# aledima00/sldm-gnn

Measured on NVIDIA B200. Metric: sageblock_fwd_bwd_edges_per_sec, higher is better.
Workload: dtype f32

## Files before the change

### include/sldm_sage.h

```cpp
#ifndef SLDM_SAGE_H_
#define SLDM_SAGE_H_

#include <stddef.h>
#include <stdint.h>

#ifdef __cplusplus
extern "C" {
#endif

#define SLDM_ABI_VERSION 1

#define SLDM_OK            0
#define SLDM_EINVAL        1
#define SLDM_ESHAPE        2
#define SLDM_ECUDA         3
#define SLDM_EWORKSPACE    4
#define SLDM_EUNSUPPORTED  5
#define SLDM_ENODEVICE     6

typedef void* sldm_stream_t;

int         sldm_abi_version(void);
const char* sldm_last_error(void);
int64_t     sldm_launch_count(void);
int         sldm_device_sm_count(int* out_sms);

#define SLDM_HUB_DEGREE 256
#define SLDM_HUB_CHUNK  2048

enum {
  SLDM_CSR_META = 0, SLDM_CSR_ROWPTR_DST = 1, SLDM_CSR_COL_SRC = 2,
  SLDM_CSR_ROWPTR_SRC = 3, SLDM_CSR_COL_DST = 4, SLDM_CSR_HUB_DST = 5,
  SLDM_CSR_HUB_SRC = 6, SLDM_CSR_TOTAL = 7
};
int     sldm_csr_layout(int64_t N, int64_t E, int64_t* out8);
int64_t sldm_csr_workspace_bytes(int64_t N, int64_t E);
int     sldm_csr_build(const int64_t* edge_index, int64_t E, int64_t N,
                       int32_t* csr, void* workspace, int64_t workspace_bytes,
                       sldm_stream_t stream);

int     sldm_csr_status_async(const int32_t* csr, int32_t* status_host_pinned, sldm_stream_t stream);

int     sldm_csr_build_pairs(const int64_t* edge_src, const int64_t* edge_dst, int64_t E, int64_t N,
                             int32_t* csr, void* workspace, int64_t workspace_bytes,
                             sldm_stream_t stream);

int64_t sldm_segment_workspace_bytes(int64_t N, int64_t E, int32_t F);
int     sldm_segment_reduce(const float* src, int64_t N, int32_t F,
                            const int32_t* csr, int64_t E, int32_t transpose,
                            int32_t mean, const float* addend, float* out,
                            void* workspace, int64_t workspace_bytes,
                            sldm_stream_t stream);

int64_t sldm_sage_project_workspace_bytes(int64_t N, int32_t Fin, int32_t Fout);
int     sldm_sage_project_forward(const float* agg, const float* x, int64_t N,
                                  int32_t Fin, int32_t Fout,
                                  const float* W_l, const float* b_l, const float* W_r,
                                  const float* ln_w, const float* ln_b,
                                  float eps, float slope,
                                  float* out, float* xhat_out, float* rstd_out,
                                  void* workspace, int64_t workspace_bytes,
                                  sldm_stream_t stream);

int64_t sldm_sage_layer_fwd_workspace_bytes(int64_t N, int64_t E, int32_t Fin, int32_t Fout);
int     sldm_sage_layer_forward(const float* x, int64_t N, int32_t Fin, int32_t Fout,
                                const int32_t* csr, int64_t E,
                                const float* W_l, const float* b_l, const float* W_r,
                                const float* ln_w, const float* ln_b,
                                float eps, float slope,
                                float* out, float* agg, float* xhat_out, float* rstd_out,
                                void* workspace, int64_t workspace_bytes,
                                sldm_stream_t stream);

int64_t sldm_sage_layer_bwd_workspace_bytes(int64_t N, int64_t E, int32_t Fin, int32_t Fout);
int     sldm_sage_layer_backward(const float* dout, const float* x, const float* agg,
                                 const float* xhat, const float* rstd,
                                 int64_t N, int32_t Fin, int32_t Fout,
                                 const int32_t* csr, int64_t E,
                                 const float* W_l, const float* W_r,
                                 const float* ln_w, const float* ln_b, float slope,
                                 float* dx, float* dW_l, float* db_l, float* dW_r,
                                 float* dln_w, float* dln_b,
                                 float* dz, float* dagg, float* dxroot,
                                 void* workspace, int64_t workspace_bytes,
                                 sldm_stream_t stream);

#define SLDM_BWD_STAGE_LN     1
#define SLDM_BWD_STAGE_DGRAD  2
#define SLDM_BWD_STAGE_WGRAD  4
#define SLDM_BWD_STAGE_GATHER 8
#define SLDM_BWD_STAGE_ALL    15
int     sldm_sage_layer_backward_stages(const float* dout, const float* x, const float* agg,
                                        const float* xhat, const float* rstd,
                                        int64_t N, int32_t Fin, int32_t Fout,
                                        const int32_t* csr, int64_t E,
                                        const float* W_l, const float* W_r,
                                        const float* ln_w, const float* ln_b, float slope,
                                        float* dx, float* dW_l, float* db_l, float* dW_r,
                                        float* dln_w, float* dln_b,
                                        float* dz, float* dagg, float* dxroot,
                                        void* workspace, int64_t workspace_bytes,
                                        sldm_stream_t stream, int32_t stages);

int sldm_sage_bf16_supported(int32_t Fin, int32_t Fout);
int sldm_segment_mean_bf16(const void* src, int64_t N, int32_t F, const int32_t* csr, int64_t E, void* out,
                           void* workspace, int64_t workspace_bytes, sldm_stream_t stream);
int sldm_sage_project_forward_bf16(const void* agg, const void* x, int64_t N, int32_t Fin, int32_t Fout,
                                   const float* W_l, const float* b_l, const float* W_r,
                                   const float* ln_w, const float* ln_b, float eps, float slope,
                                   void* out, float* xhat_out, float* rstd_out,
                                   void* workspace, int64_t workspace_bytes, sldm_stream_t stream);
int sldm_sage_layer_forward_bf16(const void* x, int64_t N, int32_t Fin, int32_t Fout,
                                 const int32_t* csr, int64_t E,
                                 const float* W_l, const float* b_l, const float* W_r,
                                 const float* ln_w, const float* ln_b, float eps, float slope,
                                 void* out, void* agg, float* xhat_out, float* rstd_out,
                                 void* workspace, int64_t workspace_bytes, sldm_stream_t stream);
int sldm_sage_layer_backward_bf16(const float* dout, const void* x, const void* agg,
                                  const float* xhat, const float* rstd,
                                  int64_t N, int32_t Fin, int32_t Fout,
                                  const int32_t* csr, int64_t E,
                                  const float* W_l, const float* W_r,
                                  const float* ln_w, const float* ln_b, float slope,
                                  float* dx, float* dW_l, float* db_l, float* dW_r,
                                  float* dln_w, float* dln_b,
                                  float* dz, float* dagg, float* dxroot,
                                  void* workspace, int64_t workspace_bytes,
                                  sldm_stream_t stream, int32_t stages);

int64_t sldm_readout_workspace_bytes(int64_t G, int32_t F);
int     sldm_readout_forward(const float* x, int64_t N, int32_t F, const int32_t* csr, int64_t csr_nodes,
                             int64_t G, float* out_mean, float* out_max, int64_t ld, sldm_stream_t stream);
int     sldm_readout_backward(const float* x, int64_t N, int32_t F, const int64_t* batch,
                              const int32_t* csr, int64_t csr_nodes, int64_t G,
                              const float* out_max, int64_t ld_max,
                              const float* dmean, const float* dmax, int64_t ld_d,
                              float* dx, void* workspace, int64_t workspace_bytes, sldm_stream_t stream);

int sldm_concat_chunks(const void* table_dev, int64_t G, int64_t max_chunk_bytes, void* out, sldm_stream_t stream);
int sldm_collate_graph_index(const void* table_dev, const int64_t* node_ptr_dev, int64_t G, int64_t Etot,
                             int64_t max_edges, int64_t max_nodes, int64_t* edge_index_out,
                             int64_t* batch_out, sldm_stream_t stream);

int64_t sldm_map_attention_workspace_bytes(int64_t B, int32_t H);
int64_t sldm_map_grid_bytes(int64_t S);
int     sldm_map_grid_build(const float* centroids, int64_t S, void* grid, int64_t grid_bytes, sldm_stream_t stream);
int     sldm_map_attention_forward_grid(const float* pos, int64_t B, const void* grid, int64_t grid_bytes, int64_t S,
                                        const float* emb, int32_t D, int32_t K,
                                        const float* W1, const float* b1, const float* W2, const float* b2, int32_t H,
                                        float* ctx, int64_t* idx_out, float* dist_out, float* w_out,
                                        sldm_stream_t stream);
int     sldm_map_attention_forward(const float* pos, int64_t B, const float* centroids, int64_t S,
                                   const float* emb, int32_t D, int32_t K,
                                   const float* W1, const float* b1, const float* W2, const float* b2, int32_t H,
                                   float* ctx, int64_t* idx_out, float* dist_out, float* w_out,
                                   sldm_stream_t stream);
int     sldm_map_attention_backward(const float* dctx, int64_t B, const float* emb, int64_t S, int32_t D, int32_t K,
                                    const int64_t* idx, const float* dist, const float* w,
                                    const float* W1, const float* b1, const float* W2, int32_t H,
                                    const int32_t* csr, int64_t csr_nodes,
                                    float* demb, float* dW1, float* db1, float* dW2, float* db2,
                                    void* workspace, int64_t workspace_bytes, sldm_stream_t stream);

int sldm_edge_build_count(const float* x, int64_t V, int32_t T, int32_t F, float m_radius,
                          int32_t* counts, int32_t* offsets, sldm_stream_t stream);
int sldm_edge_build_fill(const float* x, int64_t V, int32_t T, int32_t F, float m_radius,
                         const int32_t* offsets, int64_t E, int64_t* edge_index, float* edge_attr,
                         sldm_stream_t stream);

int     sldm_gru_supported(int32_t T, int32_t I, int32_t H);
int     sldm_gru_stack_supported(int32_t T, int32_t I, int32_t H);
int64_t sldm_gru_partial_rows(int64_t N);
int64_t sldm_gru_partial_width(int32_t H);
int     sldm_gru_forward(const float* x, int64_t N, int32_t T, int32_t I, int32_t H,
                         const float* W_ih, const float* W_hh, const float* b_ih, const float* b_hh,
                         float* h_last, float* saved, sldm_stream_t stream);
int     sldm_gru_layer_forward(const float* x, const float* gi, int64_t N, int32_t T, int32_t I, int32_t H,
                               const float* W_ih, const float* W_hh, const float* b_ih, const float* b_hh,
                               float* h_last, float* saved, float* h_seq, sldm_stream_t stream);
int     sldm_gru_backward(const float* x, int64_t N, int32_t T, int32_t I, int32_t H, const float* W_hh,
                          const float* dh_last, const float* saved, float* dgh, float* dgi_n, float* partials,
                          int64_t partial_rows, sldm_stream_t stream);
int     sldm_gru_layer_backward(const float* x, int64_t N, int32_t T, int32_t I, int32_t H, const float* W_hh,
                                const float* dh_last, const float* dh_seq, const float* saved, float* dgh,
                                float* dgi_n, float* dgi, float* partials, int64_t partial_rows, sldm_stream_t stream);
int     sldm_gru_project_forward(const float* h_seq, int64_t rows, int32_t H, const float* W_ih, const float* b_ih,
                                 float* gi, sldm_stream_t stream);
int     sldm_gru_project_backward(const float* dgi, int64_t rows, int32_t H, const float* W_ih, float* dy,
                                  sldm_stream_t stream);
int64_t sldm_gru_wgrad_tiles(int64_t N, int32_t T);
int     sldm_gru_wgrad(const float* dgh, const float* saved, int64_t N, int32_t T, int32_t H,
                       float* partials, int64_t partial_tiles, sldm_stream_t stream);
int     sldm_gru_wgrad_strided(const float* dg, const float* a, int64_t a_stride, int64_t N, int32_t T, int32_t H,
                               float* partials, int64_t partial_tiles, sldm_stream_t stream);

int sldm_sage_block_forward_host(const float* x_h, const int64_t* edge_index_h,
                                 int64_t N, int64_t E,
                                 const int32_t* hdims, int32_t L,
                                 const float* const* params_h,
                                 float eps, float slope,
                                 float* out_h);
int sldm_sage_block_train_host(const float* x_h, const int64_t* edge_index_h,
                               int64_t N, int64_t E,
                               const int32_t* hdims, int32_t L,
                               const float* const* params_h,
                               float eps, float slope,
                               const float* dout_h,
                               float* out_h, float* dx_h, float* const* grads_h);

#ifdef __cplusplus
}
#endif
#endif
```

### sldm_gnn_b200/_lib.py

```python
from __future__ import annotations

import ctypes as C
import os

_HERE = os.path.dirname(os.path.abspath(__file__))
LIB_PATH = os.environ.get("SLDM_LIB_PATH") or os.path.join(_HERE, "lib", "libsldm_sage.so")

OK, EINVAL, ESHAPE, ECUDA, EWORKSPACE, EUNSUPPORTED, ENODEVICE = range(7)
BWD_STAGE_LN, BWD_STAGE_DGRAD, BWD_STAGE_WGRAD, BWD_STAGE_GATHER, BWD_STAGE_ALL = 1, 2, 4, 8, 15
HUB_DEGREE = 256
HUB_CHUNK = 2048
CSR_SECTIONS = ("meta", "rowptr_dst", "col_src", "rowptr_src", "col_dst", "hub_dst", "hub_src", "total")

if not os.path.exists(LIB_PATH):
    raise ImportError(
        f"{LIB_PATH} not found: build it with `python __graft_entry__.py` (or `make`) first. "
        "sldm_gnn_b200 has no CPU / PyTorch fallback for the SageBlock hot path."
    )

lib = C.CDLL(LIB_PATH)

_p = C.c_void_p
_i64 = C.c_int64
_i32 = C.c_int32
_f = C.c_float

_PROTOS = {
    "sldm_abi_version": (C.c_int, []),
    "sldm_last_error": (C.c_char_p, []),
    "sldm_launch_count": (_i64, []),
    "sldm_device_sm_count": (C.c_int, [C.POINTER(C.c_int)]),
    "sldm_csr_layout": (C.c_int, [_i64, _i64, C.POINTER(_i64)]),
    "sldm_csr_workspace_bytes": (_i64, [_i64, _i64]),
    "sldm_csr_build": (C.c_int, [_p, _i64, _i64, _p, _p, _i64, _p]),
    "sldm_csr_status_async": (C.c_int, [_p, _p, _p]),
    "sldm_csr_build_pairs": (C.c_int, [_p, _p, _i64, _i64, _p, _p, _i64, _p]),
    "sldm_segment_workspace_bytes": (_i64, [_i64, _i64, _i32]),
    "sldm_segment_reduce": (C.c_int, [_p, _i64, _i32, _p, _i64, _i32, _i32, _p, _p, _p, _i64, _p]),
    "sldm_sage_project_workspace_bytes": (_i64, [_i64, _i32, _i32]),
    "sldm_sage_project_forward": (C.c_int, [_p, _p, _i64, _i32, _i32, _p, _p, _p, _p, _p, _f, _f,
                                            _p, _p, _p, _p, _i64, _p]),
    "sldm_sage_layer_fwd_workspace_bytes": (_i64, [_i64, _i64, _i32, _i32]),
    "sldm_sage_layer_forward": (C.c_int, [_p, _i64, _i32, _i32, _p, _i64, _p, _p, _p, _p, _p, _f, _f,
                                          _p, _p, _p, _p, _p, _i64, _p]),
    "sldm_sage_layer_bwd_workspace_bytes": (_i64, [_i64, _i64, _i32, _i32]),
    "sldm_sage_layer_backward": (C.c_int, [_p, _p, _p, _p, _p, _i64, _i32, _i32, _p, _i64, _p, _p, _p, _p, _f,
                                           _p, _p, _p, _p, _p, _p, _p, _p, _p, _p, _i64, _p]),
    "sldm_sage_layer_backward_stages": (C.c_int, [_p, _p, _p, _p, _p, _i64, _i32, _i32, _p, _i64, _p, _p, _p, _p, _f,
                                                  _p, _p, _p, _p, _p, _p, _p, _p, _p, _p, _i64, _p, _i32]),
    "sldm_sage_bf16_supported": (C.c_int, [_i32, _i32]),
    "sldm_segment_mean_bf16": (C.c_int, [_p, _i64, _i32, _p, _i64, _p, _p, _i64, _p]),
    "sldm_sage_project_forward_bf16": (C.c_int, [_p, _p, _i64, _i32, _i32, _p, _p, _p, _p, _p, _f, _f,
                                                 _p, _p, _p, _p, _i64, _p]),
    "sldm_sage_layer_forward_bf16": (C.c_int, [_p, _i64, _i32, _i32, _p, _i64, _p, _p, _p, _p, _p, _f, _f,
                                               _p, _p, _p, _p, _p, _i64, _p]),
    "sldm_sage_layer_backward_bf16": (C.c_int, [_p, _p, _p, _p, _p, _i64, _i32, _i32, _p, _i64, _p, _p, _p, _p, _f,
                                                _p, _p, _p, _p, _p, _p, _p, _p, _p, _p, _i64, _p, _i32]),
    "sldm_readout_workspace_bytes": (_i64, [_i64, _i32]),
    "sldm_readout_forward": (C.c_int, [_p, _i64, _i32, _p, _i64, _i64, _p, _p, _i64, _p]),
    "sldm_readout_backward": (C.c_int, [_p, _i64, _i32, _p, _p, _i64, _i64, _p, _i64, _p, _p, _i64, _p, _p, _i64, _p]),
    "sldm_concat_chunks": (C.c_int, [_p, _i64, _i64, _p, _p]),
    "sldm_collate_graph_index": (C.c_int, [_p, _p, _i64, _i64, _i64, _i64, _p, _p, _p]),
    "sldm_map_attention_workspace_bytes": (_i64, [_i64, _i32]),
    "sldm_map_attention_forward": (C.c_int, [_p, _i64, _p, _i64, _p, _i32, _i32, _p, _p, _p, _p, _i32, _p, _p, _p, _p, _p]),
    "sldm_map_grid_bytes": (_i64, [_i64]),
    "sldm_map_grid_build": (C.c_int, [_p, _i64, _p, _i64, _p]),
    "sldm_map_attention_forward_grid": (C.c_int, [_p, _i64, _p, _i64, _i64, _p, _i32, _i32, _p, _p, _p, _p, _i32, _p, _p, _p, _p, _p]),
    "sldm_map_attention_backward": (C.c_int, [_p, _i64, _p, _i64, _i32, _i32, _p, _p, _p, _p, _p, _p, _i32, _p, _i64,
                                              _p, _p, _p, _p, _p, _p, _i64, _p]),
    "sldm_edge_build_count": (C.c_int, [_p, _i64, _i32, _i32, _f, _p, _p, _p]),
    "sldm_edge_build_fill": (C.c_int, [_p, _i64, _i32, _i32, _f, _p, _i64, _p, _p, _p]),
    "sldm_gru_supported": (C.c_int, [_i32, _i32, _i32]),
    "sldm_gru_partial_rows": (_i64, [_i64]),
    "sldm_gru_partial_width": (_i64, [_i32]),
    "sldm_gru_forward": (C.c_int, [_p, _i64, _i32, _i32, _i32, _p, _p, _p, _p, _p, _p, _p]),
    "sldm_gru_backward": (C.c_int, [_p, _i64, _i32, _i32, _i32, _p, _p, _p, _p, _p, _p, _i64, _p]),
    "sldm_gru_wgrad_tiles": (_i64, [_i64, _i32]),
    "sldm_gru_wgrad": (C.c_int, [_p, _p, _i64, _i32, _i32, _p, _i64, _p]),
    "sldm_gru_stack_supported": (C.c_int, [_i32, _i32, _i32]),
    "sldm_gru_layer_forward": (C.c_int, [_p, _p, _i64, _i32, _i32, _i32, _p, _p, _p, _p, _p, _p, _p, _p]),
    "sldm_gru_layer_backward": (C.c_int, [_p, _i64, _i32, _i32, _i32, _p, _p, _p, _p, _p, _p, _p, _p, _i64, _p]),
    "sldm_gru_project_forward": (C.c_int, [_p, _i64, _i32, _p, _p, _p, _p]),
    "sldm_gru_project_backward": (C.c_int, [_p, _i64, _i32, _p, _p, _p]),
    "sldm_gru_wgrad_strided": (C.c_int, [_p, _p, _i64, _i64, _i32, _i32, _p, _i64, _p]),
    "sldm_sage_block_forward_host": (C.c_int, [_p, _p, _i64, _i64, C.POINTER(_i32), _i32, C.POINTER(_p), _f, _f, _p]),
    "sldm_sage_block_train_host": (C.c_int, [_p, _p, _i64, _i64, C.POINTER(_i32), _i32, C.POINTER(_p), _f, _f,
                                             _p, _p, _p, C.POINTER(_p)]),
}

EXPORTS = tuple(_PROTOS)

for _name, (_res, _args) in _PROTOS.items():
    _fn = getattr(lib, _name)
    _fn.restype = _res
    _fn.argtypes = _args

if lib.sldm_abi_version() != 1:
    raise ImportError(f"{LIB_PATH}: ABI version {lib.sldm_abi_version()} != 1")


def last_error() -> str:
    msg = lib.sldm_last_error()
    return msg.decode("utf-8", "replace") if msg else ""


def check(rc: int) -> None:
    if rc == OK:
        return
    msg = last_error() or f"libsldm_sage error {rc}"
    if rc == EINVAL:
        raise ValueError(msg)
    if rc == EUNSUPPORTED:
        raise NotImplementedError(msg)
    raise RuntimeError(msg)


def csr_layout(N: int, E: int) -> dict:
    out = (_i64 * 8)()
    check(lib.sldm_csr_layout(N, E, out))
    return {k: int(out[i]) for i, k in enumerate(CSR_SECTIONS)}
```

### sldm_gnn_b200/csrc/capi.cu

```cuda
#include "common.cuh"
#include <string.h>
#include <vector>
#include <atomic>
#include <mutex>

namespace sldm {

static thread_local char g_err[512] = "";

void set_error(const char* fmt, ...) {
  va_list ap;
  va_start(ap, fmt);
  vsnprintf(g_err, sizeof(g_err), fmt, ap);
  va_end(ap);
}

int cuda_fail(cudaError_t e, const char* what) {
  set_error("CUDA error %d (%s) at %s", (int)e, cudaGetErrorString(e), what);
  if (e == cudaErrorNoDevice || e == cudaErrorInsufficientDriver) return SLDM_ENODEVICE;
  return SLDM_ECUDA;
}

static std::atomic<long long> g_launches{0};
void count_launch() { g_launches.fetch_add(1, std::memory_order_relaxed); }

int num_sms() {
  static int cached = 0;
  if (cached > 0) return cached;
  int dev = 0, sms = 0;
  if (cudaGetDevice(&dev) != cudaSuccess ||
      cudaDeviceGetAttribute(&sms, cudaDevAttrMultiProcessorCount, dev) != cudaSuccess || sms <= 0) {
    cudaGetLastError();
    return 148;
  }
  cached = sms;
  return cached;
}

}

using namespace sldm;

extern "C" int sldm_abi_version(void) { return SLDM_ABI_VERSION; }
extern "C" const char* sldm_last_error(void) { return g_err; }
extern "C" int64_t sldm_launch_count(void) { return (int64_t)g_launches.load(std::memory_order_relaxed); }

extern "C" int sldm_device_sm_count(int* out_sms) {
  SLDM_REQUIRE(out_sms != nullptr, SLDM_EINVAL, "sldm_device_sm_count: NULL");
  int dev = 0, sms = 0;
  SLDM_CUDA(cudaGetDevice(&dev));
  SLDM_CUDA(cudaDeviceGetAttribute(&sms, cudaDevAttrMultiProcessorCount, dev));
  *out_sms = sms;
  return SLDM_OK;
}

extern "C" int64_t sldm_sage_layer_fwd_workspace_bytes(int64_t N, int64_t E, int32_t Fin, int32_t Fout) {
  if (N < 0 || E < 0 || Fin < 0 || Fout < 0) return -1;
  return sldm_segment_workspace_bytes(N, E, Fin) + project_forward_ws_bytes(N, Fin, Fout);
}

extern "C" int sldm_sage_layer_forward(const float* x, int64_t N, int32_t Fin, int32_t Fout,
                                       const int32_t* csr, int64_t E,
                                       const float* W_l, const float* b_l, const float* W_r,
                                       const float* ln_w, const float* ln_b,
                                       float eps, float slope,
                                       float* out, float* agg, float* xhat_out, float* rstd_out,
                                       void* workspace, int64_t workspace_bytes,
                                       sldm_stream_t stream) {
  SLDM_REQUIRE(N >= 0 && E >= 0, SLDM_EINVAL, "sldm_sage_layer_forward: negative N or E");
  SLDM_REQUIRE(Fin >= 1 && Fout >= 1, SLDM_ESHAPE, "sldm_sage_layer_forward: Fin=%d Fout=%d", Fin, Fout);
  if (N == 0) return SLDM_OK;
  SLDM_REQUIRE(x && csr && W_l && b_l && W_r && ln_w && ln_b && out && agg, SLDM_EINVAL,
               "sldm_sage_layer_forward: NULL pointer");
  const int64_t seg_ws = sldm_segment_workspace_bytes(N, E, Fin);
  const int64_t need = seg_ws + project_forward_ws_bytes(N, Fin, Fout);
  SLDM_REQUIRE(workspace != nullptr && workspace_bytes >= need, SLDM_EWORKSPACE,
               "sldm_sage_layer_forward: workspace %lld < %lld bytes", (long long)workspace_bytes, (long long)need);
  int rc = sldm_segment_reduce(x, N, Fin, csr, E, 0, 1, nullptr, agg,
                               workspace, seg_ws, stream);
  if (rc) return rc;
  return project_forward_launch(agg, x, N, Fin, Fout, W_l, b_l, W_r, ln_w, ln_b, eps, slope,
                                out, xhat_out, rstd_out, static_cast<char*>(workspace) + seg_ws,
                                workspace_bytes - seg_ws, static_cast<cudaStream_t>(stream));
}

extern "C" int64_t sldm_sage_layer_bwd_workspace_bytes(int64_t N, int64_t E, int32_t Fin, int32_t Fout) {
  if (N < 0 || E < 0 || Fin < 0 || Fout < 0) return -1;
  return sldm_segment_workspace_bytes(N, E, Fin) + layer_backward_ws_bytes(N, Fin, Fout);
}

extern "C" int sldm_sage_layer_backward(const float* dout, const float* x, const float* agg,
                                        const float* xhat, const float* rstd,
                                        int64_t N, int32_t Fin, int32_t Fout,
                                        const int32_t* csr, int64_t E,
                                        const float* W_l, const float* W_r,
                                        const float* ln_w, const float* ln_b, float slope,
                                        float* dx, float* dW_l, float* db_l, float* dW_r,
                                        float* dln_w, float* dln_b,
                                        float* dz, float* dagg, float* dxroot,
                                        void* workspace, int64_t workspace_bytes,
                                        sldm_stream_t stream) {
  return sldm_sage_layer_backward_stages(dout, x, agg, xhat, rstd, N, Fin, Fout, csr, E, W_l, W_r, ln_w, ln_b, slope,
                                         dx, dW_l, db_l, dW_r, dln_w, dln_b, dz, dagg, dxroot, workspace,
                                         workspace_bytes, stream, SLDM_BWD_STAGE_ALL);
}

static int layer_backward_impl(const float* dout, const float* x, const float* agg,
                               const float* xhat, const float* rstd,
                               int64_t N, int32_t Fin, int32_t Fout,
                               const int32_t* csr, int64_t E,
                               const float* W_l, const float* W_r,
                               const float* ln_w, const float* ln_b, float slope,
                               float* dx, float* dW_l, float* db_l, float* dW_r,
                               float* dln_w, float* dln_b,
                               float* dz, float* dagg, float* dxroot,
                               void* workspace, int64_t workspace_bytes,
                               sldm_stream_t stream, int32_t stages, bool bf16_feats) {
  SLDM_REQUIRE(N >= 0 && E >= 0, SLDM_EINVAL, "sldm_sage_layer_backward: negative N or E");
  SLDM_REQUIRE(Fin >= 1 && Fout >= 1, SLDM_ESHAPE, "sldm_sage_layer_backward: Fin=%d Fout=%d", Fin, Fout);
  SLDM_REQUIRE(dW_l && db_l && dW_r && dln_w && dln_b, SLDM_EINVAL, "sldm_sage_layer_backward: NULL gradient output");
  const bool need_dx = dx != nullptr;
  if (N > 0) {
    SLDM_REQUIRE(dout && x && agg && xhat && rstd && csr && W_l && W_r && ln_w && ln_b && dz, SLDM_EINVAL,
                 "sldm_sage_layer_backward: NULL pointer");
    SLDM_REQUIRE(!need_dx || (dagg && dxroot), SLDM_EINVAL, "sldm_sage_layer_backward: dx needs dagg and dxroot scratch");
  }
  const int64_t seg_ws = sldm_segment_workspace_bytes(N, E, Fin);
  const int64_t need = seg_ws + layer_backward_ws_bytes(N, Fin, Fout);
  SLDM_REQUIRE(N == 0 || (workspace != nullptr && workspace_bytes >= need), SLDM_EWORKSPACE,
               "sldm_sage_layer_backward: workspace %lld < %lld bytes", (long long)workspace_bytes, (long long)need);
  cudaStream_t s = static_cast<cudaStream_t>(stream);
  const int32_t* rowptr_dst = nullptr;
  if (N > 0) rowptr_dst = csr + csr_layout(N, E).off[SLDM_CSR_ROWPTR_DST];
  int rc = layer_backward_launch(dout, x, agg, xhat, rstd, N, Fin, Fout, rowptr_dst, W_l, W_r, ln_w, ln_b, slope,
                                 need_dx, dW_l, db_l, dW_r, dln_w, dln_b, dz, dagg, dxroot,
                                 static_cast<char*>(workspace) + seg_ws, workspace_bytes - seg_ws, s, stages, bf16_feats);
  if (rc || !need_dx || N == 0 || !(stages & SLDM_BWD_STAGE_GATHER)) return rc;
  return sldm_segment_reduce(dagg, N, Fin, csr, E, 1, 0, dxroot, dx,
                             workspace, seg_ws, stream);
}

extern "C" int sldm_sage_layer_backward_stages(const float* dout, const float* x, const float* agg,
                                               const float* xhat, const float* rstd,
                                               int64_t N, int32_t Fin, int32_t Fout,
                                               const int32_t* csr, int64_t E,
                                               const float* W_l, const float* W_r,
                                               const float* ln_w, const float* ln_b, float slope,
                                               float* dx, float* dW_l, float* db_l, float* dW_r,
                                               float* dln_w, float* dln_b,
                                               float* dz, float* dagg, float* dxroot,
                                               void* workspace, int64_t workspace_bytes,
                                               sldm_stream_t stream, int32_t stages) {
  return layer_backward_impl(dout, x, agg, xhat, rstd, N, Fin, Fout, csr, E, W_l, W_r, ln_w, ln_b, slope, dx, dW_l, db_l,
                             dW_r, dln_w, dln_b, dz, dagg, dxroot, workspace, workspace_bytes, stream, stages, false);
}

extern "C" int sldm_sage_bf16_supported(int32_t Fin, int32_t Fout) {
  return (Fin % 64 == 0 && Fin >= 64 && Fin <= 128 && Fout % 32 == 0 && Fout >= 32 && Fout <= 128) ? 1 : 0;
}

extern "C" int sldm_sage_layer_forward_bf16(const void* x, int64_t N, int32_t Fin, int32_t Fout,
                                            const int32_t* csr, int64_t E,
                                            const float* W_l, const float* b_l, const float* W_r,
                                            const float* ln_w, const float* ln_b, float eps, float slope,
                                            void* out, void* agg, float* xhat_out, float* rstd_out,
                                            void* workspace, int64_t workspace_bytes, sldm_stream_t stream) {
  SLDM_REQUIRE(N >= 0 && E >= 0, SLDM_EINVAL, "sldm_sage_layer_forward_bf16: negative N or E");
  SLDM_REQUIRE(sldm_sage_bf16_supported(Fin, Fout), SLDM_EUNSUPPORTED,
               "sldm_sage_layer_forward_bf16: Fin=%d Fout=%d (needs Fin in {64,128}, Fout %% 32 == 0, Fout <= 128)", Fin, Fout);
  if (N == 0) return SLDM_OK;
  SLDM_REQUIRE(x && csr && W_l && b_l && W_r && ln_w && ln_b && out && agg, SLDM_EINVAL,
               "sldm_sage_layer_forward_bf16: NULL pointer");
  SLDM_REQUIRE(project_forward_bf16_eligible(N, Fin, Fout, agg, x, out, xhat_out), SLDM_EUNSUPPORTED,
               "sldm_sage_layer_forward_bf16: buffers must be 16-byte aligned (and SLDM_DISABLE_TC unset)");
  const int64_t seg_ws = sldm_segment_workspace_bytes(N, E, Fin);
  const int64_t need = seg_ws + project_forward_ws_bytes(N, Fin, Fout);
  SLDM_REQUIRE(workspace != nullptr && workspace_bytes >= need, SLDM_EWORKSPACE,
               "sldm_sage_layer_forward_bf16: workspace %lld < %lld bytes", (long long)workspace_bytes, (long long)need);
  int rc = sldm_segment_mean_bf16(x, N, Fin, csr, E, agg, workspace, seg_ws, stream);
  if (rc) return rc;
  return project_forward_bf16_launch(agg, x, N, Fin, Fout, W_l, b_l, W_r, ln_w, ln_b, eps, slope, out, xhat_out,
                                     rstd_out, static_cast<char*>(workspace) + seg_ws, workspace_bytes - seg_ws,
                                     static_cast<cudaStream_t>(stream));
}

extern "C" int sldm_sage_project_forward_bf16(const void* agg, const void* x, int64_t N, int32_t Fin, int32_t Fout,
                                              const float* W_l, const float* b_l, const float* W_r,
                                              const float* ln_w, const float* ln_b, float eps, float slope,
                                              void* out, float* xhat_out, float* rstd_out,
                                              void* workspace, int64_t workspace_bytes, sldm_stream_t stream) {
  SLDM_REQUIRE(sldm_sage_bf16_supported(Fin, Fout), SLDM_EUNSUPPORTED, "sldm_sage_project_forward_bf16: Fin=%d Fout=%d", Fin, Fout);
  if (N == 0) return SLDM_OK;
  SLDM_REQUIRE(agg && x && W_l && b_l && W_r && ln_w && ln_b && out, SLDM_EINVAL, "sldm_sage_project_forward_bf16: NULL pointer");
  SLDM_REQUIRE(project_forward_bf16_eligible(N, Fin, Fout, agg, x, out, xhat_out), SLDM_EUNSUPPORTED,
               "sldm_sage_project_forward_bf16: buffers must be 16-byte aligned (and SLDM_DISABLE_TC unset)");
  return project_forward_bf16_launch(agg, x, N, Fin, Fout, W_l, b_l, W_r, ln_w, ln_b, eps, slope, out, xhat_out, rstd_out,
                                     workspace, workspace_bytes, static_cast<cudaStream_t>(stream));
}

extern "C" int sldm_sage_layer_backward_bf16(const float* dout, const void* x, const void* agg,
                                             const float* xhat, const float* rstd,
                                             int64_t N, int32_t Fin, int32_t Fout,
                                             const int32_t* csr, int64_t E,
                                             const float* W_l, const float* W_r,
                                             const float* ln_w, const float* ln_b, float slope,
                                             float* dx, float* dW_l, float* db_l, float* dW_r,
                                             float* dln_w, float* dln_b,
                                             float* dz, float* dagg, float* dxroot,
                                             void* workspace, int64_t workspace_bytes,
                                             sldm_stream_t stream, int32_t stages) {
  SLDM_REQUIRE(sldm_sage_bf16_supported(Fin, Fout), SLDM_EUNSUPPORTED,
               "sldm_sage_layer_backward_bf16: Fin=%d Fout=%d (needs Fin in {64,128}, Fout %% 32 == 0, Fout <= 128)", Fin, Fout);
  return layer_backward_impl(dout, static_cast<const float*>(x), static_cast<const float*>(agg), xhat, rstd, N, Fin,
                             Fout, csr, E, W_l, W_r, ln_w, ln_b, slope, dx, dW_l, db_l, dW_r, dln_w, dln_b, dz, dagg,
                             dxroot, workspace, workspace_bytes, stream, stages, true);
}

namespace {
struct DevPool {
  struct Block { void* p; size_t bytes; int dev; };
  std::mutex mu;
  std::vector<Block> free_blocks;
  size_t kept = 0;
  static size_t cap() {
    static size_t c = [] { const char* e = getenv("SLDM_HOST_POOL_MB"); return (size_t)(e ? atoll(e) : 4096) << 20; }();
    return c;
  }
  void* take(size_t bytes, int dev, size_t* real) {
    std::lock_guard<std::mutex> g(mu);
    int best = -1;
    for (int i = 0; i < (int)free_blocks.size(); ++i)
      if (free_blocks[i].dev == dev && free_blocks[i].bytes >= bytes && free_blocks[i].bytes <= 2 * bytes + (1 << 20) &&
          (best < 0 || free_blocks[i].bytes < free_blocks[best].bytes)) best = i;
    if (best < 0) return nullptr;
    void* p = free_blocks[best].p;
    *real = free_blocks[best].bytes;
    kept -= free_blocks[best].bytes;
    free_blocks.erase(free_blocks.begin() + best);
    return p;
  }
  void give(void* p, size_t bytes, int dev) {
    std::lock_guard<std::mutex> g(mu);
    if (kept + bytes > cap()) { cudaFree(p); return; }
    free_blocks.push_back({p, bytes, dev});
    kept += bytes;
  }
};
DevPool& pool() { static DevPool* p = new DevPool; return *p; }

thread_local cudaStream_t g_host_call_stream = nullptr;

struct DevBuf {
  void* p = nullptr;
  size_t bytes = 0;
  int dev = 0;
  cudaStream_t s = nullptr;
  int alloc(int64_t n) {
    if (n <= 0) n = 256;
    bytes = (size_t)((n + 255) / 256 * 256);
    s = g_host_call_stream;
    cudaGetDevice(&dev);
    size_t real = 0;
    p = pool().take(bytes, dev, &real);
    if (p) { bytes = real; return SLDM_OK; }
    cudaError_t e = cudaMalloc(&p, bytes);
    if (e != cudaSuccess) { p = nullptr; return cuda_fail(e, "cudaMalloc"); }
    return SLDM_OK;
  }
  ~DevBuf() { if (p) { if (s) cudaStreamSynchronize(s); pool().give(p, bytes, dev); } }
  template <typename T> T* as() { return static_cast<T*>(p); }
};
}

static int block_host_impl(const float* x_h, const int64_t* ei_h, int64_t N, int64_t E,
                           const int32_t* hdims, int32_t L, const float* const* params_h,
                           float eps, float slope, const float* dout_h,
                           float* out_h, float* dx_h, float* const* grads_h, bool train) {
  SLDM_REQUIRE(N >= 0 && E >= 0 && L >= 0, SLDM_EINVAL, "sage_block_host: negative N/E/L");
  SLDM_REQUIRE(hdims != nullptr, SLDM_EINVAL, "sage_block_host: hdims is NULL");
  for (int l = 0; l <= L; ++l) SLDM_REQUIRE(hdims[l] >= 1, SLDM_ESHAPE, "sage_block_host: hdims[%d]=%d", l, hdims[l]);
  SLDM_REQUIRE(N == 0 || (x_h && out_h), SLDM_EINVAL, "sage_block_host: NULL x/out");
  SLDM_REQUIRE(E == 0 || ei_h, SLDM_EINVAL, "sage_block_host: NULL edge_index");
  SLDM_REQUIRE(L == 0 || params_h, SLDM_EINVAL, "sage_block_host: NULL params");
  SLDM_REQUIRE(!train || (dout_h || N == 0), SLDM_EINVAL, "sage_block_host: NULL dout");
  SLDM_REQUIRE(!train || L == 0 || grads_h, SLDM_EINVAL, "sage_block_host: NULL grads");
  int ndev = 0;
  {
    cudaError_t e = cudaGetDeviceCount(&ndev);
    if (e != cudaSuccess || ndev == 0) {
      cudaGetLastError();
      set_error("sage_block_host: no CUDA device (there is no CPU fallback)");
      return SLDM_ENODEVICE;
    }
  }
  if (L == 0) {
    if (N > 0 && out_h != x_h) memcpy(out_h, x_h, (size_t)N * hdims[0] * 4);
    if (train && dx_h && N > 0) memcpy(dx_h, dout_h, (size_t)N * hdims[0] * 4);
    return SLDM_OK;
  }
  cudaStream_t s = nullptr;
  SLDM_CUDA(cudaStreamCreateWithFlags(&s, cudaStreamNonBlocking));
  struct StreamGuard { cudaStream_t s; ~StreamGuard() { g_host_call_stream = nullptr; cudaStreamDestroy(s); } } guard{s};
  g_host_call_stream = s;

  int Fmax = 0;
  for (int l = 0; l <= L; ++l) Fmax = hdims[l] > Fmax ? hdims[l] : Fmax;
  CsrLayout CL = csr_layout(N, E);
  int rc;
  DevBuf d_ei, d_csr, d_ws;
  if ((rc = d_ei.alloc(2 * E * 8))) return rc;
  if ((rc = d_csr.alloc(CL.off[SLDM_CSR_TOTAL] * 4))) return rc;
  int64_t ws_bytes = sldm_csr_workspace_bytes(N, E);
  for (int l = 0; l < L; ++l) {
    int64_t a = sldm_sage_layer_fwd_workspace_bytes(N, E, hdims[l], hdims[l + 1]);
    int64_t b = train ? sldm_sage_layer_bwd_workspace_bytes(N, E, hdims[l], hdims[l + 1]) : 0;
    ws_bytes = a > ws_bytes ? a : ws_bytes;
    ws_bytes = b > ws_bytes ? b : ws_bytes;
  }
  if ((rc = d_ws.alloc(ws_bytes))) return rc;
  if (E > 0) SLDM_CUDA(cudaMemcpyAsync(d_ei.p, ei_h, (size_t)2 * E * 8, cudaMemcpyHostToDevice, s));
  if ((rc = sldm_csr_build(d_ei.as<int64_t>(), E, N, d_csr.as<int32_t>(), d_ws.p, ws_bytes, s))) return rc;

  std::vector<DevBuf> act(L + 1), agg(L), xhat(train ? L : 0), rstd(train ? L : 0), par(5 * L);
  for (int l = 0; l <= L; ++l) if ((rc = act[l].alloc(N * (int64_t)hdims[l] * 4))) return rc;
  if (N > 0) SLDM_CUDA(cudaMemcpyAsync(act[0].p, x_h, (size_t)N * hdims[0] * 4, cudaMemcpyHostToDevice, s));
  for (int l = 0; l < L; ++l) {
    const int Fin = hdims[l], Fout = hdims[l + 1];
    const int64_t sizes[5] = {(int64_t)Fout * Fin, Fout, (int64_t)Fout * Fin, Fout, Fout};
    for (int k = 0; k < 5; ++k) {
      SLDM_REQUIRE(params_h[5 * l + k] != nullptr, SLDM_EINVAL, "sage_block_host: params[%d] is NULL", 5 * l + k);
      if ((rc = par[5 * l + k].alloc(sizes[k] * 4))) return rc;
      SLDM_CUDA(cudaMemcpyAsync(par[5 * l + k].p, params_h[5 * l + k], (size_t)sizes[k] * 4, cudaMemcpyHostToDevice, s));
    }
    if ((rc = agg[l].alloc(N * (int64_t)Fin * 4))) return rc;
    if (train) {
      if ((rc = xhat[l].alloc(N * (int64_t)Fout * 4))) return rc;
      if ((rc = rstd[l].alloc(N * 4))) return rc;
    }
    rc = sldm_sage_layer_forward(act[l].as<float>(), N, Fin, Fout, d_csr.as<int32_t>(), E,
                                 par[5 * l].as<float>(), par[5 * l + 1].as<float>(), par[5 * l + 2].as<float>(),
                                 par[5 * l + 3].as<float>(), par[5 * l + 4].as<float>(), eps, slope,
                                 act[l + 1].as<float>(), agg[l].as<float>(),
                                 train ? xhat[l].as<float>() : nullptr, train ? rstd[l].as<float>() : nullptr,
                                 d_ws.p, ws_bytes, s);
    if (rc) return rc;
  }
  if (N > 0) SLDM_CUDA(cudaMemcpyAsync(out_h, act[L].p, (size_t)N * hdims[L] * 4, cudaMemcpyDeviceToHost, s));

  if (train) {
    DevBuf g_cur, g_next, dz, dagg, dxroot;
    if ((rc = g_cur.alloc(N * (int64_t)Fmax * 4))) return rc;
    if ((rc = g_next.alloc(N * (int64_t)Fmax * 4))) return rc;
    if ((rc = dz.alloc(N * (int64_t)Fmax * 4))) return rc;
    if ((rc = dagg.alloc(N * (int64_t)Fmax * 4))) return rc;
    if ((rc = dxroot.alloc(N * (int64_t)Fmax * 4))) return rc;
    if (N > 0) SLDM_CUDA(cudaMemcpyAsync(g_cur.p, dout_h, (size_t)N * hdims[L] * 4, cudaMemcpyHostToDevice, s));
    std::vector<DevBuf> gpar(5 * L);
    for (int l = L - 1; l >= 0; --l) {
      const int Fin = hdims[l], Fout = hdims[l + 1];
      const int64_t sizes[5] = {(int64_t)Fout * Fin, Fout, (int64_t)Fout * Fin, Fout, Fout};
      for (int k = 0; k < 5; ++k) if ((rc = gpar[5 * l + k].alloc(sizes[k] * 4))) return rc;
      const bool need_dx = (l > 0) || (dx_h != nullptr);
      rc = sldm_sage_layer_backward(g_cur.as<float>(), act[l].as<float>(), agg[l].as<float>(),
                                    xhat[l].as<float>(), rstd[l].as<float>(), N, Fin, Fout,
                                    d_csr.as<int32_t>(), E, par[5 * l].as<float>(), par[5 * l + 2].as<float>(),
                                    par[5 * l + 3].as<float>(), par[5 * l + 4].as<float>(), slope,
                                    need_dx ? g_next.as<float>() : nullptr,
                                    gpar[5 * l].as<float>(), gpar[5 * l + 1].as<float>(), gpar[5 * l + 2].as<float>(),
                                    gpar[5 * l + 3].as<float>(), gpar[5 * l + 4].as<float>(),
                                    dz.as<float>(), dagg.as<float>(), dxroot.as<float>(), d_ws.p, ws_bytes, s);
      if (rc) return rc;
      for (int k = 0; k < 5; ++k) {
        SLDM_REQUIRE(grads_h[5 * l + k] != nullptr, SLDM_EINVAL, "sage_block_host: grads[%d] is NULL", 5 * l + k);
        SLDM_CUDA(cudaMemcpyAsync(grads_h[5 * l + k], gpar[5 * l + k].p, (size_t)sizes[k] * 4, cudaMemcpyDeviceToHost, s));
      }
      std::swap(g_cur.p, g_next.p);
    }
    if (dx_h && N > 0) SLDM_CUDA(cudaMemcpyAsync(dx_h, g_cur.p, (size_t)N * hdims[0] * 4, cudaMemcpyDeviceToHost, s));
    SLDM_CUDA(cudaStreamSynchronize(s));
    return SLDM_OK;
  }
  SLDM_CUDA(cudaStreamSynchronize(s));
  return SLDM_OK;
}

extern "C" int sldm_sage_block_forward_host(const float* x_h, const int64_t* edge_index_h,
                                            int64_t N, int64_t E,
                                            const int32_t* hdims, int32_t L,
                                            const float* const* params_h,
                                            float eps, float slope, float* out_h) {
  return block_host_impl(x_h, edge_index_h, N, E, hdims, L, params_h, eps, slope, nullptr, out_h,
                         nullptr, nullptr, false);
}

extern "C" int sldm_sage_block_train_host(const float* x_h, const int64_t* edge_index_h,
                                          int64_t N, int64_t E,
                                          const int32_t* hdims, int32_t L,
                                          const float* const* params_h,
                                          float eps, float slope, const float* dout_h,
                                          float* out_h, float* dx_h, float* const* grads_h) {
  return block_host_impl(x_h, edge_index_h, N, E, hdims, L, params_h, eps, slope, dout_h, out_h,
                         dx_h, grads_h, true);
}
```

### sldm_gnn_b200/csrc/common.cuh

```cuda
#pragma once
#include <cuda_runtime.h>
#include <stdint.h>
#include <stdio.h>
#include <stdarg.h>
#include <stdlib.h>
#include "../../include/sldm_sage.h"

namespace sldm {

void set_error(const char* fmt, ...);
int  cuda_fail(cudaError_t e, const char* what);
void count_launch();

#define SLDM_CUDA(expr)                                                \
  do {                                                                 \
    cudaError_t _e = (expr);                                           \
    if (_e != cudaSuccess) return ::sldm::cuda_fail(_e, #expr);        \
  } while (0)

#define SLDM_LAUNCH_CHECK(name)                                        \
  do {                                                                 \
    ::sldm::count_launch();                                            \
    cudaError_t _e = cudaGetLastError();                               \
    if (_e != cudaSuccess) return ::sldm::cuda_fail(_e, name);         \
  } while (0)

#define SLDM_REQUIRE(cond, code, ...)                                  \
  do {                                                                 \
    if (!(cond)) { ::sldm::set_error(__VA_ARGS__); return (code); }    \
  } while (0)

template <typename T>
__host__ __device__ constexpr T ceil_div(T a, T b) { return (a + b - 1) / b; }
template <typename T>
__host__ __device__ constexpr T round_up(T a, T b) { return ceil_div(a, b) * b; }

constexpr int64_t kAlignI32 = 64;
inline int64_t align_i32(int64_t n) { return round_up<int64_t>(n, kAlignI32); }
inline int64_t align_bytes(int64_t n) { return round_up<int64_t>(n, 256); }

int num_sms();

#define SLDM_OPT_IN_SMEM(kernel, bytes)                                                                   \
  do {                                                                                                    \
    static unsigned long long _done_mask = 0ull;    \
    int _dev = 0;                                                                                         \
    SLDM_CUDA(cudaGetDevice(&_dev));                                                                      \
    const unsigned long long _bit = 1ull << (_dev & 63);                                                  \
    if (!(_done_mask & _bit)) {                                                                           \
      SLDM_CUDA(cudaFuncSetAttribute(kernel, cudaFuncAttributeMaxDynamicSharedMemorySize, (int)(bytes))); \
      _done_mask |= _bit;                                                                                 \
    }                                                                                                     \
  } while (0)

struct Arena {
  char* base; int64_t size; int64_t off;
  Arena(void* p, int64_t n) : base(static_cast<char*>(p)), size(n), off(0) {}
  template <typename T> T* take(int64_t count) {
    int64_t bytes = align_bytes(count * (int64_t)sizeof(T));
    if (off + bytes > size) { off = size + 1; return nullptr; }
    T* r = reinterpret_cast<T*>(base + off); off += bytes; return r;
  }
  bool ok() const { return off <= size; }
};

struct CsrLayout { int64_t off[8]; };
CsrLayout csr_layout(int64_t N, int64_t E);
inline int64_t hub_capacity(int64_t E) {
  return E / SLDM_HUB_CHUNK + E / SLDM_HUB_DEGREE + 2;
}

int segment_reduce_launch(const float* src, int64_t N, int32_t F,
                          const int32_t* rowptr, const int32_t* col,
                          const int32_t* hub_list, const int32_t* hub_count, int64_t hub_cap,
                          bool mean, const float* addend, float* out,
                          float* partials, cudaStream_t s);

int project_forward_launch(const float* agg, const float* x, int64_t N, int32_t Fin, int32_t Fout,
                           const float* W_l, const float* b_l, const float* W_r,
                           const float* ln_w, const float* ln_b, float eps, float slope,
                           float* out, float* xhat, float* rstd,
                           void* ws, int64_t ws_bytes, cudaStream_t s);
int64_t project_forward_ws_bytes(int64_t N, int32_t Fin, int32_t Fout);
bool project_forward_tc_eligible(int64_t N, int32_t Fin, int32_t Fout, const float* agg, const float* x,
                                 const float* out, const float* xhat);
int64_t project_forward_tc_ws_bytes(int32_t Fin, int32_t Fout);
int project_forward_tc_launch(const float* agg, const float* x, int64_t N, int32_t Fin, int32_t Fout,
                              const float* W_l, const float* b_l, const float* W_r,
                              const float* ln_w, const float* ln_b, float eps, float slope,
                              float* out, float* xhat, float* rstd, void* ws, int64_t ws_bytes, cudaStream_t s);

int layer_backward_launch(const float* dout, const float* x, const float* agg,
                          const float* xhat, const float* rstd,
                          int64_t N, int32_t Fin, int32_t Fout,
                          const int32_t* rowptr_dst,
                          const float* W_l, const float* W_r,
                          const float* ln_w, const float* ln_b, float slope,
                          bool need_dx,
                          float* dW_l, float* db_l, float* dW_r, float* dln_w, float* dln_b,
                          float* dz, float* dagg, float* dxroot,
                          void* ws, int64_t ws_bytes, cudaStream_t s, int stages = SLDM_BWD_STAGE_ALL,
                          bool bf16_feats = false);
int64_t layer_backward_ws_bytes(int64_t N, int32_t Fin, int32_t Fout);

bool dgrad_tc_eligible(int64_t N, int32_t Fin, int32_t Fout, const float* dz, const float* dagg, const float* dxroot);
int64_t dgrad_tc_ws_bytes(int32_t Fin, int32_t Fout);
int dgrad_tc_launch(const float* dz, int64_t N, int32_t Fin, int32_t Fout, const float* W_l, const float* W_r,
                    const int32_t* rowptr_dst, float* dagg, float* dxroot, void* ws, int64_t ws_bytes,
                    cudaStream_t s);

bool wgrad_tc_eligible(int64_t N, int32_t Fin, int32_t Fout, const float* dz, const float* agg, const float* x);
int64_t wgrad_tc_ws_bytes(int32_t Fin, int32_t Fout);
int wgrad_tc_launch(const float* dz, const void* agg, const void* x, int64_t N, int32_t Fin, int32_t Fout,
                    float* part, int* nparts, cudaStream_t s, bool bf16_ops = false);
bool wgrad_bf16_eligible(int64_t N, int32_t Fin, int32_t Fout, const float* dz, const void* agg, const void* x);
bool project_forward_bf16_eligible(int64_t N, int32_t Fin, int32_t Fout, const void* agg, const void* x,
                                   const void* out, const float* xhat);
int project_forward_bf16_launch(const void* agg, const void* x, int64_t N, int32_t Fin, int32_t Fout,
                                const float* W_l, const float* b_l, const float* W_r,
                                const float* ln_w, const float* ln_b, float eps, float slope,
                                void* out, float* xhat, float* rstd, void* ws, int64_t ws_bytes, cudaStream_t s);

__device__ __forceinline__ int block_exclusive_scan_256(int v, int& total, int* smem) {
  const int lane = threadIdx.x & 31, warp = threadIdx.x >> 5;
  int inc = v;
#pragma unroll
  for (int o = 1; o < 32; o <<= 1) {
    const int t = __shfl_up_sync(0xffffffffu, inc, o);
    if (lane >= o) inc += t;
  }
  if (lane == 31) smem[warp] = inc;
  __syncthreads();
  if (warp == 0) {
    const int w = lane < 8 ? smem[lane] : 0;
    int winc = w;
#pragma unroll
    for (int o = 1; o < 8; o <<= 1) {
      const int t = __shfl_up_sync(0xffffffffu, winc, o);
      if (lane >= o) winc += t;
    }
    if (lane < 8) smem[lane] = winc - w;
    if (lane == 7) smem[8] = winc;
  }
  __syncthreads();
  const int prefix = smem[warp] + inc - v;
  total = smem[8];
  __syncthreads();
  return prefix;
}

__device__ __forceinline__ uint32_t bf16_rn(float f) {
  uint32_t u = __float_as_uint(f);
  if ((u & 0x7F800000u) == 0x7F800000u) return (u >> 16) | ((u & 0xFFFFu) ? 0x40u : 0u);
  return (u + 0x7FFFu + ((u >> 16) & 1u)) >> 16;
}
__device__ __forceinline__ uint32_t pack2_bf16(float lo, float hi) { return bf16_rn(lo) | (bf16_rn(hi) << 16); }

__device__ __forceinline__ float4 ldg4(const float* p) {
  return __ldg(reinterpret_cast<const float4*>(p));
}
__device__ __forceinline__ void st4(float* p, float4 v) {
  *reinterpret_cast<float4*>(p) = v;
}
__device__ __forceinline__ float4 f4zero() { return make_float4(0.f, 0.f, 0.f, 0.f); }
__device__ __forceinline__ void f4add(float4& a, const float4& b) {
  a.x += b.x; a.y += b.y; a.z += b.z; a.w += b.w;
}

}
```

### sldm_gnn_b200/csrc/sage_bwd.cu

```cuda
#include "common.cuh"
#include <algorithm>

namespace sldm {

constexpr int kBKb = 16;

__device__ __forceinline__ float f4at(const float4& v, int k) {
  return k == 0 ? v.x : (k == 1 ? v.y : (k == 2 ? v.z : v.w));
}

template <int TX, int TN, int TM>
struct BTile {
  static constexpr int TY = 256 / TX;
  static constexpr int BN = TX * TN;
  static constexpr int BM = TY * TM;
  __device__ static __forceinline__ int rowl(int ty, int i) {
    return (TM % 4 == 0) ? (i / 4) * (TY * 4) + ty * 4 + (i % 4) : ty * TM + i;
  }
  __device__ static __forceinline__ int coll(int tx, int j) {
    return (j / 4) * (TX * 4) + tx * 4 + (j % 4);
  }
};

constexpr int kQMax = 8;

template <int TX, int TN, int TM>
__global__ void __launch_bounds__(256)
k_ln_bwd_dgrad(const float* __restrict__ dout, const float* __restrict__ xhat,
               const float* __restrict__ rstd, const float* __restrict__ gamma,
               const float* __restrict__ beta, float slope,
               int64_t N, int Fin, int Fout, int KP,
               const float* __restrict__ W_l, const float* __restrict__ W_r,
               const int32_t* __restrict__ rowptr_dst,
               float* __restrict__ dz, float* __restrict__ dagg, float* __restrict__ dxroot,
               float* __restrict__ colpart, int need_dx, int vec_w, int vec_o) {
  using T = BTile<TX, TN, TM>;
  constexpr int BM = T::BM, BN = T::BN;
  constexpr int W_F4 = kBKb * (BN / 4);
  constexpr int W_PT = (W_F4 + 255) / 256;
  extern __shared__ __align__(16) float smem[];
  const int AZS = KP + 4;
  float* Az = smem;
  float* Ws = smem + (size_t)BM * AZS;

  const int tid = threadIdx.x, lane = tid & 31, warp = tid >> 5;
  const int tx = tid % TX, ty = tid / TX;
  const int Q = (Fout + 31) / 32;
  const float fF = (float)Fout;

  float g[kQMax], be[kQMax], pg[kQMax], pb[kQMax], pdb[kQMax];
#pragma unroll
  for (int q = 0; q < kQMax; ++q) {
    const int c = lane + 32 * q;
    const bool cv = q < Q && c < Fout;
    g[q] = cv ? __ldg(gamma + c) : 0.f;
    be[q] = cv ? __ldg(beta + c) : 0.f;
    pg[q] = pb[q] = pdb[q] = 0.f;
  }

  const int64_t ntiles = ceil_div<int64_t>(N, BM);
  for (int64_t tile = blockIdx.x; tile < ntiles; tile += gridDim.x) {
    const int64_t row0 = tile * BM;
    for (int r = warp; r < BM; r += 8) {
      const int64_t row = row0 + r;
      float* az = Az + (size_t)r * AZS;
      if (row < N) {
        const float rs = __ldg(rstd + row);
        float dzh[kQMax], xh[kQMax];
        float s1 = 0.f, s2 = 0.f;
#pragma unroll
        for (int q = 0; q < kQMax; ++q) {
          const int c = lane + 32 * q;
          dzh[q] = 0.f; xh[q] = 0.f;
          if (q < Q && c < Fout) {
            const float d = __ldg(dout + row * Fout + c);
            const float h = __ldg(xhat + row * Fout + c);
            const float y = fmaf(h, g[q], be[q]);
            const float dy = y > 0.f ? d : d * slope;
            pg[q] = fmaf(dy, h, pg[q]);
            pb[q] += dy;
            const float t = dy * g[q];
            dzh[q] = t; xh[q] = h;
            s1 += t;
            s2 = fmaf(t, h, s2);
          }
        }
#pragma unroll
        for (int o = 16; o > 0; o >>= 1) {
          s1 += __shfl_xor_sync(0xffffffffu, s1, o);
          s2 += __shfl_xor_sync(0xffffffffu, s2, o);
        }
        const float c1 = __fdiv_rn(s1, fF), c2 = __fdiv_rn(s2, fF);
#pragma unroll
        for (int q = 0; q < kQMax; ++q) {
          const int c = lane + 32 * q;
          if (q < Q && c < KP) {
            float v = 0.f;
            if (c < Fout) {
              v = rs * (dzh[q] - c1 - xh[q] * c2);
              pdb[q] += v;
              dz[row * Fout + c] = v;
            }
            az[c] = v;
          }
        }
      } else {
#pragma unroll
        for (int q = 0; q < kQMax; ++q) {
          const int c = lane + 32 * q;
          if (q < Q && c < KP) az[c] = 0.f;
        }
      }
    }
    __syncthreads();
    if (!need_dx) { __syncthreads(); continue; }

    const int nkc = KP / kBKb;
    const int nnb = (Fin + BN - 1) / BN;
    for (int pass = 0; pass < 2; ++pass) {
      const float* __restrict__ W = pass == 0 ? W_l : W_r;
      float* __restrict__ O = pass == 0 ? dagg : dxroot;
      for (int nb = 0; nb < nnb; ++nb) {
        const int n0 = nb * BN;
        float acc[TM][TN];
#pragma unroll
        for (int i = 0; i < TM; ++i)
#pragma unroll
          for (int j = 0; j < TN; ++j) acc[i][j] = 0.f;
        float4 rw[W_PT];
        auto fetch = [&](int kc) {
#pragma unroll
          for (int i = 0; i < W_PT; ++i) {
            const int f = tid + i * 256;
            if (f < W_F4) {
              const int k = kc * kBKb + f / (BN / 4);
              const int n = n0 + (f % (BN / 4)) * 4;
              float4 v = f4zero();
              if (k < Fout && n < Fin) {
                const float* p = W + (int64_t)k * Fin + n;
                if (vec_w) v = ldg4(p);
                else {
                  v.x = __ldg(p);
                  v.y = (n + 1 < Fin) ? __ldg(p + 1) : 0.f;
                  v.z = (n + 2 < Fin) ? __ldg(p + 2) : 0.f;
                  v.w = (n + 3 < Fin) ? __ldg(p + 3) : 0.f;
                }
              }
              rw[i] = v;
            }
          }
        };
        auto stash = [&](int buf) {
#pragma unroll
          for (int i = 0; i < W_PT; ++i) {
            const int f = tid + i * 256;
            if (f < W_F4) st4(Ws + (size_t)buf * kBKb * BN + (size_t)f * 4, rw[i]);
          }
        };
        fetch(0);
        stash(0);
        __syncthreads();
        for (int kc = 0; kc < nkc; ++kc) {
          const int buf = kc & 1;
          if (kc + 1 < nkc) fetch(kc + 1);
          const float* wsb = Ws + (size_t)buf * kBKb * BN;
#pragma unroll
          for (int k4 = 0; k4 < kBKb; k4 += 4) {
            float4 a[TM];
#pragma unroll
            for (int i = 0; i < TM; ++i)
              a[i] = *reinterpret_cast<const float4*>(Az + (size_t)T::rowl(ty, i) * AZS + kc * kBKb + k4);
#pragma unroll
            for (int kk = 0; kk < 4; ++kk) {
              float4 w[TN / 4];
#pragma unroll
              for (int j4 = 0; j4 < TN / 4; ++j4)
                w[j4] = *reinterpret_cast<const float4*>(wsb + (k4 + kk) * BN + T::coll(tx, j4 * 4));
#pragma unroll
              for (int i = 0; i < TM; ++i) {
                const float av = f4at(a[i], kk);
#pragma unroll
                for (int j4 = 0; j4 < TN / 4; ++j4) {
                  acc[i][j4 * 4 + 0] = fmaf(av, w[j4].x, acc[i][j4 * 4 + 0]);
                  acc[i][j4 * 4 + 1] = fmaf(av, w[j4].y, acc[i][j4 * 4 + 1]);
                  acc[i][j4 * 4 + 2] = fmaf(av, w[j4].z, acc[i][j4 * 4 + 2]);
                  acc[i][j4 * 4 + 3] = fmaf(av, w[j4].w, acc[i][j4 * 4 + 3]);
                }
              }
            }
          }
          if (kc + 1 < nkc) stash(buf ^ 1);
          __syncthreads();
        }
#pragma unroll
        for (int i = 0; i < TM; ++i) {
          const int64_t row = row0 + T::rowl(ty, i);
          if (row >= N) continue;
          float inv_cnt = 1.f;
          if (pass == 0) {
            int deg = __ldg(rowptr_dst + row + 1) - __ldg(rowptr_dst + row);
            deg = deg < 1 ? 1 : (deg > 16777216 ? 16777216 : deg);
            inv_cnt = (float)deg;
          }
          float* orow = O + row * Fin;
#pragma unroll
          for (int j4 = 0; j4 < TN / 4; ++j4) {
            const int n = n0 + T::coll(tx, j4 * 4);
            float o[4];
#pragma unroll
            for (int q = 0; q < 4; ++q)
              o[q] = pass == 0 ? __fdiv_rn(acc[i][j4 * 4 + q], inv_cnt) : acc[i][j4 * 4 + q];
            if (vec_o) { if (n < Fin) st4(orow + n, make_float4(o[0], o[1], o[2], o[3])); }
            else {
#pragma unroll
              for (int q = 0; q < 4; ++q) if (n + q < Fin) orow[n + q] = o[q];
            }
          }
        }
      }
    }
    __syncthreads();
  }

  __syncthreads();
  float* cp = smem;
  const int CW = 32 * Q;
#pragma unroll
  for (int q = 0; q < kQMax; ++q) {
    if (q < Q) {
      cp[(warp * 3 + 0) * CW + lane + 32 * q] = pg[q];
      cp[(warp * 3 + 1) * CW + lane + 32 * q] = pb[q];
      cp[(warp * 3 + 2) * CW + lane + 32 * q] = pdb[q];
    }
  }
  __syncthreads();
  for (int idx = tid; idx < 3 * Fout; idx += 256) {
    const int which = idx / Fout, c = idx % Fout;
    float s = 0.f;
#pragma unroll
    for (int w = 0; w < 8; ++w) s += cp[(w * 3 + which) * CW + c];
    colpart[(int64_t)blockIdx.x * 3 * Fout + idx] = s;
  }
}

template <int VPL>
__global__ void __launch_bounds__(256)
k_ln_bwd_rows(const float* __restrict__ dout, const float* __restrict__ xhat, const float* __restrict__ rstd,
              const float* __restrict__ gamma, const float* __restrict__ beta, float slope,
              int64_t N, int Fout, float* __restrict__ dz, float* __restrict__ colpart) {
  constexpr int R = 4;
  __shared__ float cp[8][3][128 * VPL];
  const int tid = threadIdx.x, lane = tid & 31, warp = tid >> 5;
  const float fF = (float)Fout;
  float4 g[VPL], be[VPL], pg[VPL], pb[VPL], pdb[VPL];
  bool cv[VPL];
#pragma unroll
  for (int q = 0; q < VPL; ++q) {
    const int c = (lane + 32 * q) * 4;
    cv[q] = c < Fout;
    g[q] = cv[q] ? ldg4(gamma + c) : f4zero();
    be[q] = cv[q] ? ldg4(beta + c) : f4zero();
    pg[q] = pb[q] = pdb[q] = f4zero();
  }
  const int64_t nwarps = (int64_t)gridDim.x * 8;
  for (int64_t r0 = ((int64_t)blockIdx.x * 8 + warp) * R; r0 < N; r0 += nwarps * R) {
    float4 d[R][VPL], h[R][VPL];
    float rs[R];
#pragma unroll
    for (int i = 0; i < R; ++i) {
      const int64_t row = r0 + i;
      const bool rv = row < N;
      rs[i] = rv ? __ldg(rstd + row) : 0.f;
#pragma unroll
      for (int q = 0; q < VPL; ++q) {
        const bool v = rv && cv[q];
        d[i][q] = v ? ldg4(dout + row * Fout + (lane + 32 * q) * 4) : f4zero();
        h[i][q] = v ? ldg4(xhat + row * Fout + (lane + 32 * q) * 4) : f4zero();
      }
    }
#pragma unroll
    for (int i = 0; i < R; ++i) {
      const int64_t row = r0 + i;
      float s1 = 0.f, s2 = 0.f;
      float4 t[VPL];
#pragma unroll
      for (int q = 0; q < VPL; ++q) {
        const float* dd = reinterpret_cast<const float*>(&d[i][q]);
        const float* hh = reinterpret_cast<const float*>(&h[i][q]);
        const float* gg = reinterpret_cast<const float*>(&g[q]);
        const float* bb = reinterpret_cast<const float*>(&be[q]);
        float* tt = reinterpret_cast<float*>(&t[q]);
        float* ppg = reinterpret_cast<float*>(&pg[q]);
        float* ppb = reinterpret_cast<float*>(&pb[q]);
#pragma unroll
        for (int e = 0; e < 4; ++e) {
          const float y = fmaf(hh[e], gg[e], bb[e]);
          const float dy = y > 0.f ? dd[e] : dd[e] * slope;
          ppg[e] = fmaf(dy, hh[e], ppg[e]);
          ppb[e] += dy;
          tt[e] = dy * gg[e];
          s1 += tt[e];
          s2 = fmaf(tt[e], hh[e], s2);
        }
      }
#pragma unroll
      for (int o = 16; o > 0; o >>= 1) {
        s1 += __shfl_xor_sync(0xffffffffu, s1, o);
        s2 += __shfl_xor_sync(0xffffffffu, s2, o);
      }
      const float c1 = __fdiv_rn(s1, fF), c2 = __fdiv_rn(s2, fF);
      if (row < N) {
#pragma unroll
        for (int q = 0; q < VPL; ++q) {
          if (cv[q]) {
            const float* hh = reinterpret_cast<const float*>(&h[i][q]);
            const float* tt = reinterpret_cast<const float*>(&t[q]);
            float* pp = reinterpret_cast<float*>(&pdb[q]);
            float4 o4;
            float* oo = reinterpret_cast<float*>(&o4);
#pragma unroll
            for (int e = 0; e < 4; ++e) {
              oo[e] = rs[i] * (tt[e] - c1 - hh[e] * c2);
              pp[e] += oo[e];
            }
            st4(dz + row * Fout + (lane + 32 * q) * 4, o4);
          }
        }
      }
    }
  }
#pragma unroll
  for (int q = 0; q < VPL; ++q) {
    const int c = (lane + 32 * q) * 4;
    st4(&cp[warp][0][c], pg[q]);
    st4(&cp[warp][1][c], pb[q]);
    st4(&cp[warp][2][c], pdb[q]);
  }
  __syncthreads();
  for (int idx = tid; idx < 3 * Fout; idx += 256) {
    const int which = idx / Fout, c = idx % Fout;
    float s = 0.f;
#pragma unroll
    for (int w = 0; w < 8; ++w) s += cp[w][which][c];
    colpart[(int64_t)blockIdx.x * 3 * Fout + idx] = s;
  }
}

__global__ void __launch_bounds__(256)
k_wgrad(const float* __restrict__ dz, const float* __restrict__ agg, const float* __restrict__ x,
        int64_t N, int Fin, int Fout, int64_t rows_per_slab, int MB, int NB,
        float* __restrict__ part, int vec_m, int vec_n) {
  __shared__ __align__(16) float As[2][kBKb][128];
  __shared__ __align__(16) float Bs[2][kBKb][128];
  const int tid = threadIdx.x, tn = tid % 16, tm = tid / 16;
  const int s = blockIdx.x;
  int t = blockIdx.y;
  const int nb = t % NB; t /= NB;
  const int mb = t % MB; t /= MB;
  const int which = t;
  const float* __restrict__ B = which == 0 ? agg : x;
  const int m0 = mb * 128, n0 = nb * 128;
  const int64_t r0 = (int64_t)s * rows_per_slab;
  const int64_t r1 = (r0 + rows_per_slab < N) ? r0 + rows_per_slab : N;

  float acc[8][8];
#pragma unroll
  for (int i = 0; i < 8; ++i)
#pragma unroll
    for (int j = 0; j < 8; ++j) acc[i][j] = 0.f;

  float4 ra[2], rb[2];
  auto ld_guard = [&](const float* __restrict__ P, int64_t row, int ld, int c, int cmax, int vec) -> float4 {
    float4 v = f4zero();
    if (row < r1 && c < cmax) {
      const float* p = P + row * ld + c;
      if (vec) v = ldg4(p);
      else {
        v.x = __ldg(p);
        v.y = (c + 1 < cmax) ? __ldg(p + 1) : 0.f;
        v.z = (c + 2 < cmax) ? __ldg(p + 2) : 0.f;
        v.w = (c + 3 < cmax) ? __ldg(p + 3) : 0.f;
      }
    }
    return v;
  };
  auto fetch = [&](int64_t rc) {
#pragma unroll
    for (int i = 0; i < 2; ++i) {
      const int f = tid + i * 256;
      const int k = f / 32, c4 = (f % 32) * 4;
      ra[i] = ld_guard(dz, rc + k, Fout, m0 + c4, Fout, vec_m);
      rb[i] = ld_guard(B, rc + k, Fin, n0 + c4, Fin, vec_n);
    }
  };
  auto stash = [&](int buf) {
#pragma unroll
    for (int i = 0; i < 2; ++i) {
      const int f = tid + i * 256;
      st4(&As[buf][0][0] + f * 4, ra[i]);
      st4(&Bs[buf][0][0] + f * 4, rb[i]);
    }
  };
  const int64_t nch = r1 > r0 ? ceil_div<int64_t>(r1 - r0, kBKb) : 0;
  if (nch > 0) {
    fetch(r0);
    stash(0);
  }
  __syncthreads();
  for (int64_t ch = 0; ch < nch; ++ch) {
    const int buf = (int)(ch & 1);
    if (ch + 1 < nch) fetch(r0 + (ch + 1) * kBKb);
#pragma unroll
    for (int k = 0; k < kBKb; ++k) {
      const float4 a0 = *reinterpret_cast<const float4*>(&As[buf][k][tm * 4]);
      const float4 a1 = *reinterpret_cast<const float4*>(&As[buf][k][64 + tm * 4]);
      const float4 b0 = *reinterpret_cast<const float4*>(&Bs[buf][k][tn * 4]);
      const float4 b1 = *reinterpret_cast<const float4*>(&Bs[buf][k][64 + tn * 4]);
      const float av[8] = {a0.x, a0.y, a0.z, a0.w, a1.x, a1.y, a1.z, a1.w};
      const float bv[8] = {b0.x, b0.y, b0.z, b0.w, b1.x, b1.y, b1.z, b1.w};
#pragma unroll
      for (int i = 0; i < 8; ++i)
#pragma unroll
        for (int j = 0; j < 8; ++j) acc[i][j] = fmaf(av[i], bv[j], acc[i][j]);
    }
    if (ch + 1 < nch) stash(buf ^ 1);
    __syncthreads();
  }
  float* P = part + ((int64_t)s * 2 + which) * Fout * Fin;
#pragma unroll
  for (int i = 0; i < 8; ++i) {
    const int m = m0 + (i / 4) * 64 + tm * 4 + (i % 4);
    if (m >= Fout) continue;
#pragma unroll
    for (int j = 0; j < 8; ++j) {
      const int n = n0 + (j / 4) * 64 + tn * 4 + (j % 4);
      if (n < Fin) P[(int64_t)m * Fin + n] = acc[i][j];
    }
  }
}

__global__ void __launch_bounds__(256)
k_reduce_parts(const float* __restrict__ part, int S, int64_t stride, int64_t count,
               float* __restrict__ out0, int64_t split, float* __restrict__ out1,
               int64_t split2, float* __restrict__ out2) {
  __shared__ float sm[8][32];
  const int lane = threadIdx.x & 31, w = threadIdx.x >> 5;
  const int64_t i = (int64_t)blockIdx.x * 32 + lane;
  float s = 0.f;
  if (i < count)
    for (int k = w; k < S; k += 8) s += __ldg(part + (int64_t)k * stride + i);
  sm[w][lane] = s;
  __syncthreads();
  if (w == 0 && i < count) {
    float t = sm[0][lane];
#pragma unroll
    for (int q = 1; q < 8; ++q) t += sm[q][lane];
    if (i < split) out0[i] = t;
    else if (i < split2) out1[i - split] = t;
    else out2[i - split2] = t;
  }
}

struct BwdPlan { int grid1; int grid_ln; int S; int64_t rows_per_slab; int MB, NB; int64_t colpart_off, part_off, tc_off, wg_off, total; };

static BwdPlan bwd_plan(int64_t N, int Fin, int Fout) {
  BwdPlan p;
  const int sms = num_sms();
  const int64_t ntiles = ceil_div<int64_t>(N > 0 ? N : 1, 64);
  p.grid1 = (int)std::min<int64_t>(ntiles, (int64_t)sms * 2);
  p.MB = ceil_div(Fout, 128);
  p.NB = ceil_div(Fin, 128);
  const int per = 2 * p.MB * p.NB;
  const int target = std::max(1, 4 * sms / per);
  p.S = (int)std::max<int64_t>(1, std::min<int64_t>(ceil_div<int64_t>(N > 0 ? N : 1, 128), target));
  p.rows_per_slab = round_up<int64_t>(ceil_div<int64_t>(N > 0 ? N : 1, p.S), kBKb);
  p.S = (int)ceil_div<int64_t>(N > 0 ? N : 1, p.rows_per_slab);
  int64_t o = 0;
  p.grid_ln = (int)std::min<int64_t>(ceil_div<int64_t>(N > 0 ? N : 1, 32), (int64_t)sms * 4);
  p.colpart_off = o; o += align_bytes((int64_t)std::max(p.grid1, p.grid_ln) * 3 * Fout * 4);
  p.part_off = o;    o += align_bytes((int64_t)p.S * 2 * Fout * Fin * 4);
  p.tc_off = o;      o += dgrad_tc_ws_bytes(Fin, Fout);
  p.wg_off = o;      o += wgrad_tc_ws_bytes(Fin, Fout);
  p.total = o;
  return p;
}

int64_t layer_backward_ws_bytes(int64_t N, int32_t Fin, int32_t Fout) {
  return bwd_plan(N, Fin, Fout).total;
}

static bool b16(const void* p) { return (reinterpret_cast<uintptr_t>(p) & 15u) == 0; }

template <int TX, int TN, int TM>
static int launch_b1(int grid, size_t smem, cudaStream_t s,
                     const float* dout, const float* xhat, const float* rstd, const float* gamma,
                     const float* beta, float slope, int64_t N, int Fin, int Fout, int KP,
                     const float* W_l, const float* W_r, const int32_t* rowptr_dst,
                     float* dz, float* dagg, float* dxroot, float* colpart, int need_dx, int vec_w, int vec_o) {
  SLDM_OPT_IN_SMEM((k_ln_bwd_dgrad<TX, TN, TM>), 160 * 1024);
  k_ln_bwd_dgrad<TX, TN, TM><<<grid, 256, smem, s>>>(dout, xhat, rstd, gamma, beta, slope, N, Fin, Fout, KP,
                                                     W_l, W_r, rowptr_dst, dz, dagg, dxroot, colpart,
                                                     need_dx, vec_w, vec_o);
  SLDM_LAUNCH_CHECK("k_ln_bwd_dgrad");
  return SLDM_OK;
}

int layer_backward_launch(const float* dout, const float* x, const float* agg,
                          const float* xhat, const float* rstd,
                          int64_t N, int32_t Fin, int32_t Fout,
                          const int32_t* rowptr_dst,
                          const float* W_l, const float* W_r,
                          const float* ln_w, const float* ln_b, float slope,
                          bool need_dx,
                          float* dW_l, float* db_l, float* dW_r, float* dln_w, float* dln_b,
                          float* dz, float* dagg, float* dxroot,
                          void* ws, int64_t ws_bytes, cudaStream_t s, int stages, bool bf16_feats) {
  SLDM_REQUIRE(Fin >= 1 && Fout >= 1, SLDM_ESHAPE, "backward: Fin=%d Fout=%d must be >= 1", Fin, Fout);
  SLDM_REQUIRE(!bf16_feats || N == 0 || (wgrad_bf16_eligible(N, Fin, Fout, dz, agg, x) &&
                                         (!need_dx || dgrad_tc_eligible(N, Fin, Fout, dz, dagg, dxroot))),
               SLDM_EUNSUPPORTED, "backward (bf16 features): needs Fin %% 64 == 0, Fin <= 128, Fout %% 32 == 0, Fout <= 128");
  SLDM_REQUIRE(Fout <= 256, SLDM_EUNSUPPORTED, "backward: Fout=%d > 256 is not covered by the kernels", Fout);
  const int64_t wcount = (int64_t)Fout * Fin;
  if (N == 0) {
    SLDM_CUDA(cudaMemsetAsync(dW_l, 0, wcount * 4, s));
    SLDM_CUDA(cudaMemsetAsync(dW_r, 0, wcount * 4, s));
    SLDM_CUDA(cudaMemsetAsync(db_l, 0, Fout * 4, s));
    SLDM_CUDA(cudaMemsetAsync(dln_w, 0, Fout * 4, s));
    SLDM_CUDA(cudaMemsetAsync(dln_b, 0, Fout * 4, s));
    return SLDM_OK;
  }
  BwdPlan p = bwd_plan(N, Fin, Fout);
  SLDM_REQUIRE(ws != nullptr && ws_bytes >= p.total, SLDM_EWORKSPACE, "backward: workspace %lld < %lld bytes",
               (long long)ws_bytes, (long long)p.total);
  float* colpart = reinterpret_cast<float*>(static_cast<char*>(ws) + p.colpart_off);
  float* part = reinterpret_cast<float*>(static_cast<char*>(ws) + p.part_off);

  const int KP = round_up<int>(Fout, kBKb);
  const int vec_w = (Fin % 4 == 0) && b16(W_l) && b16(W_r);
  const int vec_o = (Fin % 4 == 0) && b16(dagg) && b16(dxroot);
  const int bn = Fin <= 32 ? 32 : (Fin <= 64 ? 64 : (Fin <= 96 ? 96 : 128));
  const int Q = ceil_div(Fout, 32);
  size_t smem_az = (size_t)64 * (KP + 4) * 4;
  size_t smem_cp = (size_t)8 * 3 * 32 * Q * 4;
  size_t smem = std::max(smem_az, smem_cp) + (size_t)2 * kBKb * bn * 4;
  const bool tc_dgrad = need_dx && dgrad_tc_eligible(N, Fin, Fout, dz, dagg, dxroot);
  const bool simt_dx = need_dx && !tc_dgrad;
  int rc = SLDM_OK;
  int ncolparts = p.grid1;
  const bool ln_stream = !simt_dx && (Fout % 4 == 0) && b16(dout) && b16(xhat) && b16(dz) && b16(ln_w) && b16(ln_b);
  if (!(stages & SLDM_BWD_STAGE_LN)) {
    ncolparts = ln_stream ? p.grid_ln : p.grid1;
  } else if (ln_stream) {
    ncolparts = p.grid_ln;
    if (Fout <= 128)
      k_ln_bwd_rows<1><<<p.grid_ln, 256, 0, s>>>(dout, xhat, rstd, ln_w, ln_b, slope, N, Fout, dz, colpart);
    else
      k_ln_bwd_rows<2><<<p.grid_ln, 256, 0, s>>>(dout, xhat, rstd, ln_w, ln_b, slope, N, Fout, dz, colpart);
    SLDM_LAUNCH_CHECK("k_ln_bwd_rows");
  } else {
#define SLDM_B1(TX, TN, TM) \
  rc = launch_b1<TX, TN, TM>(p.grid1, smem, s, dout, xhat, rstd, ln_w, ln_b, slope, N, Fin, Fout, KP, W_l, W_r, \
                             rowptr_dst, dz, dagg, dxroot, colpart, simt_dx ? 1 : 0, vec_w, vec_o)
  switch (bn) {
    case 32: SLDM_B1(8, 4, 2); break;
    case 64: SLDM_B1(16, 4, 4); break;
    case 96: SLDM_B1(8, 12, 2); break;
    default: SLDM_B1(16, 8, 4); break;
  }
#undef SLDM_B1
  }
  if (rc) return rc;
  if (tc_dgrad && (stages & SLDM_BWD_STAGE_DGRAD)) {
    rc = dgrad_tc_launch(dz, N, Fin, Fout, W_l, W_r, rowptr_dst, dagg, dxroot, static_cast<char*>(ws) + p.tc_off,
                         p.total - p.tc_off, s);
    if (rc) return rc;
  }

  if (!(stages & SLDM_BWD_STAGE_WGRAD)) return SLDM_OK;
  int nparts = p.S;
  if (bf16_feats || wgrad_tc_eligible(N, Fin, Fout, dz, agg, x)) {
    part = reinterpret_cast<float*>(static_cast<char*>(ws) + p.wg_off);
    if ((rc = wgrad_tc_launch(dz, agg, x, N, Fin, Fout, part, &nparts, s, bf16_feats))) return rc;
  } else {
    dim3 grid(p.S, 2 * p.MB * p.NB);
    const int vec_m = (Fout % 4 == 0) && b16(dz);
    const int vec_n = (Fin % 4 == 0) && b16(agg) && b16(x);
    k_wgrad<<<grid, 256, 0, s>>>(dz, agg, x, N, Fin, Fout, p.rows_per_slab, p.MB, p.NB, part, vec_m, vec_n);
    SLDM_LAUNCH_CHECK("k_wgrad");
  }
  {
    const int64_t count = 2 * wcount;
    k_reduce_parts<<<(unsigned)ceil_div<int64_t>(count, 32), 256, 0, s>>>(part, nparts, 2 * wcount, count,
                                                                         dW_l, wcount, dW_r, count, nullptr);
    SLDM_LAUNCH_CHECK("k_reduce_parts(dW)");
    const int64_t c3 = 3 * (int64_t)Fout;
    k_reduce_parts<<<(unsigned)ceil_div<int64_t>(c3, 32), 256, 0, s>>>(colpart, ncolparts, c3, c3,
                                                                      dln_w, Fout, dln_b, 2 * (int64_t)Fout, db_l);
    SLDM_LAUNCH_CHECK("k_reduce_parts(cols)");
  }
  return SLDM_OK;
}

}
```

### sldm_gnn_b200/csrc/segment_reduce.cu

```cuda
#include "common.cuh"
#include <algorithm>
#include <type_traits>

namespace sldm {

template <typename VT> struct Vec;
template <> struct Vec<float4> {
  static __device__ __forceinline__ float4 zero() { return make_float4(0.f, 0.f, 0.f, 0.f); }
  static __device__ __forceinline__ float4 ld(const float4* p) { return __ldg(p); }
  static __device__ __forceinline__ void add(float4& a, const float4& b) { a.x += b.x; a.y += b.y; a.z += b.z; a.w += b.w; }
  static __device__ __forceinline__ float4 div(const float4& a, float c) {
    return make_float4(__fdiv_rn(a.x, c), __fdiv_rn(a.y, c), __fdiv_rn(a.z, c), __fdiv_rn(a.w, c));
  }
};
template <> struct Vec<float> {
  static __device__ __forceinline__ float zero() { return 0.f; }
  static __device__ __forceinline__ float ld(const float* p) { return __ldg(p); }
  static __device__ __forceinline__ void add(float& a, const float& b) { a += b; }
  static __device__ __forceinline__ float div(const float& a, float c) { return __fdiv_rn(a, c); }
};

__device__ __forceinline__ float ref_count(int deg) {
  int c = deg < 1 ? 1 : (deg > 16777216 ? 16777216 : deg);
  return (float)c;
}

template <typename VT, int LPR, int VPL, int UNR>
__device__ __forceinline__ void accumulate_range(const VT* __restrict__ src, int64_t FV, int fv0,
                                                 const int32_t* __restrict__ col, int beg, int end,
                                                 int lig, unsigned gmask, VT (&acc)[VPL]) {
  bool act[VPL];
#pragma unroll
  for (int q = 0; q < VPL; ++q) act[q] = (int64_t)fv0 + lig + q * LPR < FV;
  for (int k = beg; k < end; k += LPR) {
    const int nk = min(LPR, end - k);
    const int mycol = (lig < nk) ? __ldg(col + k + lig) : 0;
    for (int j = 0; j < nk; j += UNR) {
      VT v[UNR][VPL];
#pragma unroll
      for (int u = 0; u < UNR; ++u) {
        const int c = __shfl_sync(gmask, mycol, j + u, LPR);
        const bool ok = (j + u) < nk;
        const VT* p = src + (int64_t)c * FV + fv0 + lig;
#pragma unroll
        for (int q = 0; q < VPL; ++q) v[u][q] = (ok && act[q]) ? Vec<VT>::ld(p + q * LPR) : Vec<VT>::zero();
      }
#pragma unroll
      for (int u = 0; u < UNR; ++u) {
#pragma unroll
        for (int q = 0; q < VPL; ++q) Vec<VT>::add(acc[q], v[u][q]);
      }
    }
  }
}

template <int LPR>
__device__ __forceinline__ unsigned group_mask(int lane) {
  if constexpr (LPR == 32) {
    return 0xffffffffu;
  } else {
    return ((1u << LPR) - 1u) << ((lane / LPR) * LPR);
  }
}

constexpr int kRowsPerCta = 256;

template <typename VT, int LPR, int VPL, int UNR>
__global__ void __launch_bounds__(256)
k_segment_rows(const VT* __restrict__ src, int64_t FV,
               const int32_t* __restrict__ rowptr, const int32_t* __restrict__ col,
               int64_t N, int mean, const VT* __restrict__ addend, VT* __restrict__ out) {
  constexpr int RPW = 32 / LPR;
  constexpr int STEP = 8 * RPW;
  const int lane = threadIdx.x & 31;
  const int lig = lane % LPR;
  const unsigned gmask = group_mask<LPR>(lane);
  const int64_t base = (int64_t)blockIdx.x * kRowsPerCta + (threadIdx.x >> 5) * RPW + lane / LPR;
  for (int off = 0; off < kRowsPerCta; off += STEP) {
    const int64_t row = base + off;
    if (row >= N) break;
    const int beg = __ldg(rowptr + row), end = __ldg(rowptr + row + 1);
    const int deg = end - beg;
    if (deg > SLDM_HUB_DEGREE) continue;
    const float cnt = ref_count(deg);
    for (int64_t fv0 = 0; fv0 < FV; fv0 += LPR * VPL) {
      VT acc[VPL];
#pragma unroll
      for (int q = 0; q < VPL; ++q) acc[q] = Vec<VT>::zero();
      accumulate_range<VT, LPR, VPL, UNR>(src, FV, (int)fv0, col, beg, end, lig, gmask, acc);
#pragma unroll
      for (int q = 0; q < VPL; ++q) {
        const int64_t idx = fv0 + lig + q * LPR;
        if (idx < FV) {
          VT r = acc[q];
          if (mean) r = Vec<VT>::div(r, cnt);
          if (addend) { VT a = Vec<VT>::ld(addend + row * FV + idx); Vec<VT>::add(a, r); r = a; }
          out[row * FV + idx] = r;
        }
      }
    }
  }
}

__device__ __forceinline__ int ldg_stream_i32(const int32_t* p) {
  int v;
  asm volatile("ld.global.nc.L1::no_allocate.b32 %0, [%1];" : "=r"(v) : "l"(p));
  return v;
}
__device__ __forceinline__ float4 ldg_stream_f4(const float4* p) {
  float4 v;
  asm volatile("ld.global.nc.L1::no_allocate.v4.f32 {%0, %1, %2, %3}, [%4];"
               : "=f"(v.x), "=f"(v.y), "=f"(v.z), "=f"(v.w) : "l"(p));
  return v;
}

__device__ __forceinline__ const float4* row_ptr(const char* __restrict__ pb, int c, int row_bytes) {
  return reinterpret_cast<const float4*>(pb + (int64_t)c * row_bytes);
}
template <int U>
__device__ __forceinline__ void gather_piece(const char* __restrict__ pb, int row_bytes, const int* w, float4& acc) {
  float4 v[U];
#pragma unroll
  for (int u = 0; u < U; ++u) v[u] = __ldg(row_ptr(pb, w[u], row_bytes));
#pragma unroll
  for (int u = 0; u < U; ++u) { acc.x += v[u].x; acc.y += v[u].y; acc.z += v[u].z; acc.w += v[u].w; }
}

template <int LPR, int UMAX, int RW>
__global__ void __launch_bounds__(256)
k_segment_rows_lean(const float4* __restrict__ src, int64_t FV,
                    const int32_t* __restrict__ rowptr, const int32_t* __restrict__ col,
                    int64_t N, int mean, const float4* __restrict__ addend, float4* __restrict__ out) {
  constexpr int rw = RW;
  constexpr int RPW = 32 / LPR;
  constexpr int CH = RPW <= 4 ? 256 * RPW : 1024;
  __shared__ int s_win[8][CH];
  const int lane = threadIdx.x & 31, warp = threadIdx.x >> 5;
  const int g = lane / LPR, lig = lane % LPR;
  int* win = s_win[warp];
  const int64_t wbase = ((int64_t)blockIdx.x * 8 + warp) * rw;
  if (wbase >= N) return;
  const int64_t wend = (wbase + rw < N) ? wbase + rw : N;
  const int64_t myrow = (wbase + lane < wend) ? wbase + lane : wend;
  const int rb = __ldg(rowptr + myrow);
  const int re = __ldg(rowptr + (myrow + 1 < wend ? myrow + 1 : wend));
  const int e_last = __shfl_sync(0xffffffffu, re, 31);
  const bool cvalid = lig < FV;
  const char* __restrict__ pb = reinterpret_cast<const char*>(src + (cvalid ? lig : 0));
  const int row_bytes = (int)FV * 16;
  int ws = -CH - 1;
#pragma unroll 1
  for (int it = 0; it < rw / RPW; ++it) {
    const int rfirst = it * RPW;
    if (wbase + rfirst >= wend) break;
    const int ibeg = __shfl_sync(0xffffffffu, rb, rfirst);
    const int iend = __shfl_sync(0xffffffffu, re, rfirst + RPW - 1);
    if (iend > ws + CH) {
      __syncwarp();
      ws = ibeg;
#pragma unroll
      for (int q = 0; q < CH / 32; ++q) {
        const int e = ws + lane + 32 * q;
        if (e < e_last) win[lane + 32 * q] = ldg_stream_i32(col + e);
      }
      __syncwarp();
    }
    const int beg = __shfl_sync(0xffffffffu, rb, rfirst + g);
    const int end = __shfl_sync(0xffffffffu, re, rfirst + g);
    const int64_t row = wbase + rfirst + g;
    const int deg = end - beg;
    if (row >= wend || deg > SLDM_HUB_DEGREE) continue;
    float4 acc = make_float4(0.f, 0.f, 0.f, 0.f);
    if (beg >= ws && end <= ws + CH) {
      const int* w = win + (beg - ws);
      int rem = deg;
      if constexpr (UMAX >= 8) {
        for (; rem >= 8; rem -= 8, w += 8) gather_piece<8>(pb, row_bytes, w, acc);
        if (rem >= 4) { gather_piece<4>(pb, row_bytes, w, acc); rem -= 4; w += 4; }
      } else {
        for (; rem >= 4; rem -= 4, w += 4) gather_piece<4>(pb, row_bytes, w, acc);
      }
      if (rem >= 2) { gather_piece<2>(pb, row_bytes, w, acc); rem -= 2; w += 2; }
      if (rem >= 1) gather_piece<1>(pb, row_bytes, w, acc);
    } else {
#pragma unroll 1
      for (int k = beg; k < end; ++k) {
        const float4 v = __ldg(row_ptr(pb, __ldg(col + k), row_bytes));
        acc.x += v.x; acc.y += v.y; acc.z += v.z; acc.w += v.w;
      }
    }
    if (cvalid) {
      if (mean && deg > 1) {
        if ((deg & (deg - 1)) == 0) {
          const float rc = __fdiv_rn(1.f, (float)deg);
          acc.x *= rc; acc.y *= rc; acc.z *= rc; acc.w *= rc;
        } else {
          acc = Vec<float4>::div(acc, ref_count(deg));
        }
      }
      if (addend != nullptr) { float4 a = ldg_stream_f4(addend + row * FV + lig); Vec<float4>::add(a, acc); acc = a; }
      out[row * FV + lig] = acc;
    }
  }
}

template <typename VT, int LPR, int VPL, int UNR>
__global__ void __launch_bounds__(256)
k_segment_hub_chunks(const VT* __restrict__ src, int64_t FV,
                     const int32_t* __restrict__ rowptr, const int32_t* __restrict__ col,
                     const int4* __restrict__ hub_list, const int32_t* __restrict__ hub_count,
                     int cap, VT* __restrict__ partials) {
  constexpr int G = 256 / LPR;
  constexpr int PER = SLDM_HUB_CHUNK / G;
  __shared__ VT sm[G][LPR * VPL];
  const int n = min(*hub_count, cap);
  const int lane = threadIdx.x & 31;
  const int g = threadIdx.x / LPR, lig = threadIdx.x % LPR;
  const unsigned gmask = group_mask<LPR>(lane);
  for (int c = blockIdx.x; c < n; c += gridDim.x) {
    const int4 ent = hub_list[c];
    const int rbeg = __ldg(rowptr + ent.x), rend = __ldg(rowptr + ent.x + 1);
    const int cb = rbeg + ent.y * SLDM_HUB_CHUNK;
    const int ce = min(rend, cb + SLDM_HUB_CHUNK);
    const int b = min(ce, cb + g * PER), e = min(ce, b + PER);
    for (int64_t fv0 = 0; fv0 < FV; fv0 += LPR * VPL) {
      VT acc[VPL];
#pragma unroll
      for (int q = 0; q < VPL; ++q) acc[q] = Vec<VT>::zero();
      accumulate_range<VT, LPR, VPL, UNR>(src, FV, (int)fv0, col, b, e, lig, gmask, acc);
#pragma unroll
      for (int q = 0; q < VPL; ++q) sm[g][lig + q * LPR] = acc[q];
      __syncthreads();
      if (threadIdx.x < LPR * VPL) {
        const int64_t idx = fv0 + threadIdx.x;
        if (idx < FV) {
          VT s = sm[0][threadIdx.x];
#pragma unroll 4
          for (int gg = 1; gg < G; ++gg) Vec<VT>::add(s, sm[gg][threadIdx.x]);
          partials[(int64_t)c * FV + idx] = s;
        }
      }
      __syncthreads();
    }
  }
}

template <typename VT, int LPR>
__global__ void __launch_bounds__(256)
k_segment_hub_finalize(const VT* __restrict__ partials, int64_t FV,
                       const int32_t* __restrict__ rowptr,
                       const int4* __restrict__ hub_list, const int32_t* __restrict__ hub_count,
                       int cap, int mean, const VT* __restrict__ addend, VT* __restrict__ out) {
  const int n = min(*hub_count, cap);
  const int64_t groups = (int64_t)gridDim.x * (256 / LPR);
  const int lig = threadIdx.x % LPR;
  for (int64_t c = (int64_t)blockIdx.x * (256 / LPR) + threadIdx.x / LPR; c < n; c += groups) {
    const int4 ent = hub_list[c];
    if (ent.y != 0) continue;
    const int64_t row = ent.x;
    const float cnt = ref_count(__ldg(rowptr + row + 1) - __ldg(rowptr + row));
    for (int64_t idx = lig; idx < FV; idx += LPR) {
      VT s = partials[c * FV + idx];
      for (int j = 1; j < ent.z; ++j) Vec<VT>::add(s, partials[(c + j) * FV + idx]);
      if (mean) s = Vec<VT>::div(s, cnt);
      if (addend) { VT a = Vec<VT>::ld(addend + row * FV + idx); Vec<VT>::add(a, s); s = a; }
      out[row * FV + idx] = s;
    }
  }
}

template <typename VT, int LPR, int VPL, int UNR>
static int launch_all(const float* src, int64_t N, int64_t FV,
                      const int32_t* rowptr, const int32_t* col,
                      const int32_t* hub_list, const int32_t* hub_count, int64_t hub_cap,
                      bool mean, const float* addend, float* out, float* partials, cudaStream_t s) {
  const VT* vsrc = reinterpret_cast<const VT*>(src);
  const VT* vadd = reinterpret_cast<const VT*>(addend);
  VT* vout = reinterpret_cast<VT*>(out);
  VT* vpart = reinterpret_cast<VT*>(partials);
  const int64_t grid = ceil_div<int64_t>(N, kRowsPerCta);
  if constexpr (std::is_same<VT, float4>::value && VPL == 1) {
    static const int lean = [] { const char* e = getenv("SLDM_SEG_LEAN"); return e ? atoi(e) : 4; }();
    constexpr int RW = (LPR == 32) ? 8 : 32;
    const int64_t lgrid = ceil_div<int64_t>(N, 8 * RW);
    if (lean == 4 || lean == 1)
      k_segment_rows_lean<LPR, 4, RW><<<(unsigned)lgrid, 256, 0, s>>>(vsrc, FV, rowptr, col, N, mean ? 1 : 0, vadd, vout);
    else if (lean != 0)
      k_segment_rows_lean<LPR, 8, RW><<<(unsigned)lgrid, 256, 0, s>>>(vsrc, FV, rowptr, col, N, mean ? 1 : 0, vadd, vout);
    else
      k_segment_rows<VT, LPR, VPL, UNR><<<(unsigned)grid, 256, 0, s>>>(vsrc, FV, rowptr, col, N, mean ? 1 : 0, vadd, vout);
  } else {
    k_segment_rows<VT, LPR, VPL, UNR><<<(unsigned)grid, 256, 0, s>>>(vsrc, FV, rowptr, col, N, mean ? 1 : 0, vadd, vout);
  }
  SLDM_LAUNCH_CHECK("k_segment_rows");
  if (hub_cap > 0 && hub_list != nullptr) {
    const int cap = (int)hub_cap;
    const int g1 = (int)std::min<int64_t>(hub_cap, (int64_t)num_sms() * 8);
    k_segment_hub_chunks<VT, LPR, VPL, UNR><<<g1, 256, 0, s>>>(
        vsrc, FV, rowptr, col, reinterpret_cast<const int4*>(hub_list), hub_count, cap, vpart);
    SLDM_LAUNCH_CHECK("k_segment_hub_chunks");
    const int g2 = (int)std::min<int64_t>(ceil_div<int64_t>(hub_cap, 256 / LPR), (int64_t)num_sms() * 4);
    k_segment_hub_finalize<VT, LPR><<<g2, 256, 0, s>>>(
        vpart, FV, rowptr, reinterpret_cast<const int4*>(hub_list), hub_count, cap, mean ? 1 : 0, vadd, vout);
    SLDM_LAUNCH_CHECK("k_segment_hub_finalize");
  }
  return SLDM_OK;
}

static bool aligned16(const void* p) { return (reinterpret_cast<uintptr_t>(p) & 15u) == 0; }

int segment_reduce_launch(const float* src, int64_t N, int32_t F,
                          const int32_t* rowptr, const int32_t* col,
                          const int32_t* hub_list, const int32_t* hub_count, int64_t hub_cap,
                          bool mean, const float* addend, float* out,
                          float* partials, cudaStream_t s) {
  if (N == 0 || F == 0) return SLDM_OK;
  const bool vec = (F % 4 == 0) && aligned16(src) && aligned16(out) && aligned16(addend) && aligned16(partials);
  if (vec) {
    const int64_t FV = F / 4;
    if (FV <= 4)  return launch_all<float4, 4, 1, 8>(src, N, FV, rowptr, col, hub_list, hub_count, hub_cap, mean, addend, out, partials, s);
    if (FV <= 8)  return launch_all<float4, 8, 1, 8>(src, N, FV, rowptr, col, hub_list, hub_count, hub_cap, mean, addend, out, partials, s);
    if (FV <= 16) return launch_all<float4, 16, 1, 8>(src, N, FV, rowptr, col, hub_list, hub_count, hub_cap, mean, addend, out, partials, s);
    if (FV <= 32) return launch_all<float4, 32, 1, 8>(src, N, FV, rowptr, col, hub_list, hub_count, hub_cap, mean, addend, out, partials, s);
    return launch_all<float4, 32, 2, 4>(src, N, FV, rowptr, col, hub_list, hub_count, hub_cap, mean, addend, out, partials, s);
  }
  if (F <= 32) return launch_all<float, 32, 1, 8>(src, N, F, rowptr, col, hub_list, hub_count, hub_cap, mean, addend, out, partials, s);
  return launch_all<float, 32, 4, 4>(src, N, F, rowptr, col, hub_list, hub_count, hub_cap, mean, addend, out, partials, s);
}

}

using namespace sldm;

extern "C" int64_t sldm_segment_workspace_bytes(int64_t N, int64_t E, int32_t F) {
  if (N < 0 || E < 0 || F < 0) return -1;
  return align_bytes(hub_capacity(E) * (int64_t)F * 4);
}

extern "C" int sldm_segment_reduce(const float* src, int64_t N, int32_t F,
                                   const int32_t* csr, int64_t E, int32_t transpose,
                                   int32_t mean, const float* addend, float* out,
                                   void* workspace, int64_t workspace_bytes,
                                   sldm_stream_t stream) {
  SLDM_REQUIRE(N >= 0 && E >= 0 && F >= 0, SLDM_EINVAL, "sldm_segment_reduce: negative size");
  SLDM_REQUIRE(csr != nullptr, SLDM_EINVAL, "sldm_segment_reduce: csr is NULL");
  SLDM_REQUIRE(N == 0 || F == 0 || (src != nullptr && out != nullptr), SLDM_EINVAL, "sldm_segment_reduce: NULL src/out");
  const int64_t need = sldm_segment_workspace_bytes(N, E, F);
  SLDM_REQUIRE(workspace_bytes >= need && (workspace != nullptr || need == 0), SLDM_EWORKSPACE,
               "sldm_segment_reduce: workspace %lld < %lld bytes", (long long)workspace_bytes, (long long)need);
  CsrLayout L = csr_layout(N, E);
  const int32_t* meta = csr + L.off[SLDM_CSR_META];
  const int32_t* rowptr = csr + L.off[transpose ? SLDM_CSR_ROWPTR_SRC : SLDM_CSR_ROWPTR_DST];
  const int32_t* col = csr + L.off[transpose ? SLDM_CSR_COL_DST : SLDM_CSR_COL_SRC];
  const int32_t* hub = csr + L.off[transpose ? SLDM_CSR_HUB_SRC : SLDM_CSR_HUB_DST];
  return segment_reduce_launch(src, N, F, rowptr, col, E > SLDM_HUB_DEGREE ? hub : nullptr,
                               meta + (transpose ? 1 : 0), E > SLDM_HUB_DEGREE ? hub_capacity(E) : 0,
                               mean != 0, addend, out, static_cast<float*>(workspace),
                               static_cast<cudaStream_t>(stream));
}
```

### sldm_gnn_b200/ops.py

```python
from __future__ import annotations

import collections
import os
import threading

import torch

from . import _lib
from ._lib import lib, check


def _stream(device) -> int:
    return torch.cuda.current_stream(device).cuda_stream


def _ptr(t) -> int | None:
    return None if t is None else t.data_ptr()


def _require_cuda(t: torch.Tensor, name: str) -> None:
    if not t.is_cuda:
        raise RuntimeError(
            f"sldm_gnn_b200: `{name}` is on {t.device}; the SageBlock hot path is CUDA only "
            "(sm_100a kernels, no CPU fallback)")


def check_edge_index(edge_index) -> None:
    if not isinstance(edge_index, torch.Tensor):
        raise ValueError("`edge_index` must be a torch.Tensor of dtype torch.long and shape [2, num_edges]")
    if edge_index.dtype != torch.long:
        raise ValueError(f"Expected 'edge_index' to be of integer type (got '{edge_index.dtype}')")
    if edge_index.dim() != 2:
        raise ValueError(f"Expected 'edge_index' to be two-dimensional (got {edge_index.dim()} dimensions)")
    if edge_index.size(0) != 2:
        raise ValueError(f"Expected 'edge_index' to have size '2' in the first dimension (got '{edge_index.size(0)}')")


class _IndexChecks:

    SLOTS = 256

    def __init__(self):
        self.lock = threading.Lock()
        self.pending = collections.deque()
        self.ring = None
        self.next = 0

    @staticmethod
    def mode() -> str:
        return os.environ.get("SLDM_CHECK_INDICES", "deferred")

    def watch(self, csr_buf: torch.Tensor, what: str) -> None:
        mode = self.mode()
        if mode == "0":
            return
        if mode == "1":
            if int(csr_buf[2]) != 0:
                raise IndexError(f"{what}: index out of range")
            return
        if torch.cuda.is_current_stream_capturing():
            return
        with self.lock:
            if self.ring is None:
                t = torch.full((self.SLOTS,), -1, dtype=torch.int32).pin_memory()
                self.ring = (t, t.numpy(), t.data_ptr())
            if len(self.pending) >= self.SLOTS - 1:
                self._drain(block=True)
            i = self.next % self.SLOTS
            self.next += 1
            self.ring[1][i] = -1
            check(lib.sldm_csr_status_async(csr_buf.data_ptr(), self.ring[2] + 4 * i, _stream(csr_buf.device)))
            self.pending.append((i, what))

    def _drain(self, block: bool) -> None:
        bad = None
        arr = self.ring[1]
        while self.pending:
            i, what = self.pending[0]
            v = int(arr[i])
            if v < 0:
                if not block:
                    break
                torch.cuda.synchronize()
                v = int(arr[i])
            self.pending.popleft()
            if v > 0 and bad is None:
                bad = what
        if bad is not None:
            raise IndexError(f"{bad}: index out of range (reported by an earlier device-side CSR build; "
                             "SLDM_CHECK_INDICES=1 raises at the call that passed it)")

    def poll(self, block: bool = False) -> None:
        if not self.pending or torch.cuda.is_current_stream_capturing():
            return
        with self.lock:
            self._drain(block)


index_checks = _IndexChecks()


class Csr:

    __slots__ = ("buf", "N", "E", "layout", "device")

    def __init__(self, buf, N, E, layout):
        self.buf, self.N, self.E, self.layout, self.device = buf, N, E, layout, buf.device

    def _view(self, name, n):
        o = self.layout[name]
        return self.buf[o:o + n]

    @property
    def meta(self): return self._view("meta", 64)
    @property
    def rowptr_dst(self): return self._view("rowptr_dst", self.N + 1)
    @property
    def col_src(self): return self._view("col_src", self.E)
    @property
    def rowptr_src(self): return self._view("rowptr_src", self.N + 1)
    @property
    def col_dst(self): return self._view("col_dst", self.E)

    def status(self) -> dict:
        m = self.meta[:5].cpu().tolist()
        return {"hub_chunks_dst": m[0], "hub_chunks_src": m[1], "index_out_of_range": bool(m[2]),
                "src_sorted": not m[3], "dst_sorted": not m[4]}


def build_csr(edge_index: torch.Tensor, num_nodes: int) -> Csr:
    check_edge_index(edge_index)
    _require_cuda(edge_index, "edge_index")
    index_checks.poll()
    ei = edge_index if edge_index.is_contiguous() else edge_index.contiguous()
    E = int(ei.size(1))
    N = int(num_nodes)
    dev = ei.device
    layout = _lib.csr_layout(N, E)
    with torch.cuda.device(dev):
        buf = torch.empty(layout["total"], dtype=torch.int32, device=dev)
        wsb = int(lib.sldm_csr_workspace_bytes(N, E))
        ws = torch.empty(wsb, dtype=torch.uint8, device=dev) if E > 0 else None
        check(lib.sldm_csr_build(_ptr(ei) if E > 0 else None, E, N, buf.data_ptr(), _ptr(ws), wsb if E > 0 else 0,
                                 _stream(dev)))
        csr = Csr(buf, N, E, layout)
        if E > 0:
            index_checks.watch(buf, f"edge_index (num_nodes = {N})")
    return csr


def segment_reduce(src: torch.Tensor, csr: Csr, *, transpose: bool = False, mean: bool = True,
                   addend: torch.Tensor | None = None) -> torch.Tensor:
    _require_cuda(src, "src")
    src = src.contiguous()
    N, F = src.shape
    if N != csr.N:
        raise RuntimeError(f"segment_reduce: src has {N} rows but the CSR was built for {csr.N} nodes")
    dev = src.device
    with torch.cuda.device(dev):
        out = torch.empty_like(src)
        wsb = int(lib.sldm_segment_workspace_bytes(N, csr.E, F))
        ws = torch.empty(max(wsb, 1), dtype=torch.uint8, device=dev)
        check(lib.sldm_segment_reduce(src.data_ptr(), N, F, csr.buf.data_ptr(), csr.E, int(transpose), int(mean),
                                      _ptr(addend), out.data_ptr(), ws.data_ptr(), wsb, _stream(dev)))
    return out


def segment_mean_bf16(src: torch.Tensor, csr: Csr) -> torch.Tensor:
    _require_cuda(src, "src")
    src = src.contiguous()
    N, F = src.shape
    dev = src.device
    with torch.cuda.device(dev):
        out = torch.empty_like(src)
        wsb = int(lib.sldm_segment_workspace_bytes(N, csr.E, F))
        ws = torch.empty(max(wsb, 1), dtype=torch.uint8, device=dev)
        check(lib.sldm_segment_mean_bf16(src.data_ptr(), N, F, csr.buf.data_ptr(), csr.E, out.data_ptr(), ws.data_ptr(),
                                         wsb, _stream(dev)))
    return out


def project_forward(agg, x, W_l, b_l, W_r, ln_w, ln_b, eps, slope, save: bool):
    N, Fin = x.shape
    Fout = W_l.shape[0]
    dev = x.device
    bf16 = x.dtype == torch.bfloat16
    with torch.cuda.device(dev):
        if bf16:
            out = torch.empty((N, Fout), dtype=torch.bfloat16, device=dev)
            xhat = torch.empty((N, Fout), dtype=torch.float32, device=dev) if save else None
            rstd = torch.empty((N,), dtype=torch.float32, device=dev) if save else None
            wsb = int(lib.sldm_sage_project_workspace_bytes(N, Fin, Fout))
            ws = torch.empty(max(wsb, 1), dtype=torch.uint8, device=dev)
            check(lib.sldm_sage_project_forward_bf16(agg.data_ptr(), x.data_ptr(), N, Fin, Fout, W_l.data_ptr(),
                                                     b_l.data_ptr(), W_r.data_ptr(), ln_w.data_ptr(), ln_b.data_ptr(),
                                                     float(eps), float(slope), out.data_ptr(), _ptr(xhat), _ptr(rstd),
                                                     ws.data_ptr(), wsb, _stream(dev)))
            return out, xhat, rstd
        out = torch.empty((N, Fout), dtype=torch.float32, device=dev)
        xhat = torch.empty((N, Fout), dtype=torch.float32, device=dev) if save else None
        rstd = torch.empty((N,), dtype=torch.float32, device=dev) if save else None
        wsb = int(lib.sldm_sage_project_workspace_bytes(N, Fin, Fout))
        ws = torch.empty(max(wsb, 1), dtype=torch.uint8, device=dev)
        check(lib.sldm_sage_project_forward(agg.data_ptr(), x.data_ptr(), N, Fin, Fout, W_l.data_ptr(), b_l.data_ptr(),
                                            W_r.data_ptr(), ln_w.data_ptr(), ln_b.data_ptr(), float(eps), float(slope),
                                            out.data_ptr(), _ptr(xhat), _ptr(rstd), ws.data_ptr(), wsb, _stream(dev)))
    return out, xhat, rstd


def bf16_supported(Fin: int, Fout: int) -> bool:
    return bool(lib.sldm_sage_bf16_supported(int(Fin), int(Fout)))


def layer_forward(x, csr: Csr, W_l, b_l, W_r, ln_w, ln_b, eps: float, slope: float, save: bool):
    N, Fin = x.shape
    Fout = W_l.shape[0]
    dev = x.device
    if x.dtype == torch.bfloat16:
        if not bf16_supported(Fin, Fout):
            x32, out, agg, xhat, rstd = layer_forward(x.float(), csr, W_l, b_l, W_r, ln_w, ln_b, eps, slope, save)
            return x32, out.to(torch.bfloat16), agg, xhat, rstd
        with torch.cuda.device(dev):
            out = torch.empty((N, Fout), dtype=torch.bfloat16, device=dev)
            agg = torch.empty((N, Fin), dtype=torch.bfloat16, device=dev)
            xhat = torch.empty((N, Fout), dtype=torch.float32, device=dev) if save else None
            rstd = torch.empty((N,), dtype=torch.float32, device=dev) if save else None
            wsb = int(lib.sldm_sage_layer_fwd_workspace_bytes(N, csr.E, Fin, Fout))
            ws = torch.empty(max(wsb, 1), dtype=torch.uint8, device=dev)
            check(lib.sldm_sage_layer_forward_bf16(x.data_ptr(), N, Fin, Fout, csr.buf.data_ptr(), csr.E,
                                                   W_l.data_ptr(), b_l.data_ptr(), W_r.data_ptr(), ln_w.data_ptr(),
                                                   ln_b.data_ptr(), float(eps), float(slope),
                                                   out.data_ptr(), agg.data_ptr(), _ptr(xhat), _ptr(rstd),
                                                   ws.data_ptr(), wsb, _stream(dev)))
        return x, out, agg, xhat, rstd
    with torch.cuda.device(dev):
        out = torch.empty((N, Fout), dtype=torch.float32, device=dev)
        agg = torch.empty((N, Fin), dtype=torch.float32, device=dev)
        xhat = torch.empty((N, Fout), dtype=torch.float32, device=dev) if save else None
        rstd = torch.empty((N,), dtype=torch.float32, device=dev) if save else None
        wsb = int(lib.sldm_sage_layer_fwd_workspace_bytes(N, csr.E, Fin, Fout))
        ws = torch.empty(max(wsb, 1), dtype=torch.uint8, device=dev)
        check(lib.sldm_sage_layer_forward(x.data_ptr(), N, Fin, Fout, csr.buf.data_ptr(), csr.E,
                                          W_l.data_ptr(), b_l.data_ptr(), W_r.data_ptr(), ln_w.data_ptr(),
                                          ln_b.data_ptr(), float(eps), float(slope),
                                          out.data_ptr(), agg.data_ptr(), _ptr(xhat), _ptr(rstd),
                                          ws.data_ptr(), wsb, _stream(dev)))
    return x, out, agg, xhat, rstd


def backward_buffers(N: int, Fin: int, Fout: int, E: int, dev, need_dx: bool, grad_out=None) -> dict:
    with torch.cuda.device(dev):
        f32 = dict(dtype=torch.float32, device=dev)
        if grad_out is not None:
            b = dict(dW_l=grad_out[0], db_l=grad_out[1], dW_r=grad_out[2], dln_w=grad_out[3], dln_b=grad_out[4])
        else:
            b = dict(dW_l=torch.empty((Fout, Fin), **f32), dW_r=torch.empty((Fout, Fin), **f32),
                     db_l=torch.empty((Fout,), **f32), dln_w=torch.empty((Fout,), **f32), dln_b=torch.empty((Fout,), **f32))
        b.update(dz=torch.empty((N, Fout), **f32), dx=None, dagg=None, dxroot=None)
        if need_dx:
            b.update(dx=torch.empty((N, Fin), **f32), dagg=torch.empty((N, Fin), **f32),
                     dxroot=torch.empty((N, Fin), **f32))
        wsb = int(lib.sldm_sage_layer_bwd_workspace_bytes(N, E, Fin, Fout))
        b["wsb"] = wsb
        b["ws"] = torch.empty(max(wsb, 1), dtype=torch.uint8, device=dev)
    return b


def layer_backward(dout, x, agg, xhat, rstd, csr: Csr, W_l, W_r, ln_w, ln_b, slope: float, need_dx: bool,
                   stages: int = _lib.BWD_STAGE_ALL, bufs: dict | None = None, on_param_grads=None, grad_out=None):
    N, Fin = x.shape
    Fout = W_l.shape[0]
    dev = x.device
    dout = dout.contiguous()
    b = bufs if bufs is not None else backward_buffers(N, Fin, Fout, csr.E, dev, need_dx, grad_out)

    entry = lib.sldm_sage_layer_backward_bf16 if x.dtype == torch.bfloat16 else lib.sldm_sage_layer_backward_stages
    if x.dtype != agg.dtype or dout.dtype != torch.float32:
        raise RuntimeError(f"layer_backward: x is {x.dtype}, agg is {agg.dtype}, dout is {dout.dtype}")

    def launch(mask):
        check(entry(
            dout.data_ptr(), x.data_ptr(), agg.data_ptr(), xhat.data_ptr(), rstd.data_ptr(), N, Fin, Fout,
            csr.buf.data_ptr(), csr.E, W_l.data_ptr(), W_r.data_ptr(), ln_w.data_ptr(), ln_b.data_ptr(), float(slope),
            _ptr(b["dx"]), b["dW_l"].data_ptr(), b["db_l"].data_ptr(), b["dW_r"].data_ptr(), b["dln_w"].data_ptr(),
            b["dln_b"].data_ptr(), b["dz"].data_ptr(), _ptr(b["dagg"]), _ptr(b["dxroot"]), b["ws"].data_ptr(), b["wsb"],
            _stream(dev), int(mask)))

    with torch.cuda.device(dev):
        if on_param_grads is not None and stages == _lib.BWD_STAGE_ALL:
            launch(_lib.BWD_STAGE_ALL & ~_lib.BWD_STAGE_GATHER)
            ev = torch.cuda.Event()
            ev.record(torch.cuda.current_stream(dev))
            on_param_grads(ev)
            if need_dx and N > 0:
                launch(_lib.BWD_STAGE_GATHER)
        else:
            launch(stages)
    return b["dx"], b["dW_l"], b["db_l"], b["dW_r"], b["dln_w"], b["dln_b"]
```

### sldm_gnn_b200/sageblock.py

```python
from __future__ import annotations

import math

import torch
from torch.autograd.function import once_differentiable
import torch.nn as nn

from . import ops


class _Linear(nn.Module):

    def __init__(self, in_channels: int, out_channels: int, bias: bool):
        super().__init__()
        self.in_channels, self.out_channels = in_channels, out_channels
        self.weight = nn.Parameter(torch.empty(out_channels, in_channels))
        if bias:
            self.bias = nn.Parameter(torch.empty(out_channels))
        else:
            self.register_parameter("bias", None)
        self.reset_parameters()

    def reset_parameters(self) -> None:
        bound = 1.0 / math.sqrt(self.in_channels) if self.in_channels > 0 else 0.0
        with torch.no_grad():
            self.weight.uniform_(-bound, bound)
            if self.bias is not None:
                self.bias.uniform_(-bound, bound)

    def extra_repr(self) -> str:
        return f"{self.in_channels}, {self.out_channels}, bias={self.bias is not None}"


class SageConvParams(nn.Module):

    def __init__(self, in_channels: int, out_channels: int):
        super().__init__()
        self.in_channels, self.out_channels = in_channels, out_channels
        self.lin_l = _Linear(in_channels, out_channels, bias=True)
        self.lin_r = _Linear(in_channels, out_channels, bias=False)

    def reset_parameters(self) -> None:
        self.lin_l.reset_parameters()
        self.lin_r.reset_parameters()

    def extra_repr(self) -> str:
        return f"{self.in_channels}, {self.out_channels}, aggr=mean"


class _SageBlockFn(torch.autograd.Function):

    @staticmethod
    def forward(ctx, x, csr, eps, slopes, drops, *params):
        L = len(params) // 5
        save = any(ctx.needs_input_grad)
        h, keep = x, []
        for l in range(L):
            W_l, b_l, W_r, ln_w, ln_b = params[5 * l:5 * l + 5]
            h, out, agg, xhat, rstd = ops.layer_forward(h, csr, W_l, b_l, W_r, ln_w, ln_b, eps[l], slopes[l], save)
            mask = None
            if drops[l] is not None:
                out, mask = torch.native_dropout(out, drops[l], True)
            if save:
                keep += [h, agg, xhat, rstd, mask]
            h = out
        if save:
            tensors = [t for t in keep if t is not None]
            ctx.layout = [t is not None for t in keep]
            ctx.save_for_backward(*tensors, *params)
            ctx.csr, ctx.slopes, ctx.drops, ctx.L = csr, slopes, drops, L
        return h

    @staticmethod
    @once_differentiable
    def backward(ctx, dout):
        L = ctx.L
        saved = list(ctx.saved_tensors)
        params = saved[len(saved) - 5 * L:]
        it = iter(saved[:len(saved) - 5 * L])
        keep = [next(it) if present else None for present in ctx.layout]
        sink = None
        if torch.distributed.is_available() and torch.distributed.is_initialized() and not torch.cuda.is_current_stream_capturing():
            from .parallel import active_wrapper
            sink = active_wrapper()
        grads = [None] * (5 * L)
        g = dout if dout.dtype == torch.float32 else dout.float()
        for l in range(L - 1, -1, -1):
            h, agg, xhat, rstd, mask = keep[5 * l:5 * l + 5]
            W_l, _, W_r, ln_w, ln_b = params[5 * l:5 * l + 5]
            if mask is not None:
                g = torch.ops.aten.native_dropout_backward(g, mask, 1.0 / (1.0 - ctx.drops[l]))
            g = g.contiguous()
            need_dx = l > 0 or ctx.needs_input_grad[0]
            claim = sink.claim(params[5 * l:5 * l + 5]) if sink is not None else None
            if claim is not None:
                bi, views = claim
                dx = ops.layer_backward(g, h, agg, xhat, rstd, ctx.csr, W_l, W_r, ln_w, ln_b, ctx.slopes[l], need_dx,
                                        grad_out=views, on_param_grads=lambda ev, bi=bi: sink.bucket_ready(bi, ev))[0]
            else:
                dx, dW_l, db_l, dW_r, dln_w, dln_b = ops.layer_backward(
                    g, h, agg, xhat, rstd, ctx.csr, W_l, W_r, ln_w, ln_b, ctx.slopes[l], need_dx)
                grads[5 * l:5 * l + 5] = [dW_l, db_l, dW_r, dln_w, dln_b]
            g = dx
        return (g, None, None, None, None, *grads)


class SageBlock(nn.Module):
    def __init__(self, hdims: list[int], dropout: float | None = None, negative_slope: float | None = None):
        super().__init__()
        assert len(hdims) >= 1, "hdims must contain at least one element"
        self.convs = nn.ModuleList([SageConvParams(hdims[i], hdims[i + 1]) for i in range(len(hdims) - 1)])
        self.posts = nn.ModuleList([
            nn.Sequential(
                nn.LayerNorm(hdims[i + 1]),
                nn.LeakyReLU(negative_slope=negative_slope) if negative_slope is not None else nn.ReLU(),
                nn.Dropout(p=dropout) if dropout is not None else nn.Identity(),
            ) for i in range(len(hdims) - 1)
        ])
        self._csr_key = None
        self._csr = None

    def _get_csr(self, edge_index: torch.Tensor, num_nodes: int) -> ops.Csr:
        try:
            version = edge_index._version
        except RuntimeError:
            version = None
        key = self._csr_key
        if (version is not None and key is not None and key[0] is edge_index and key[1] == version
                and key[2] == num_nodes):
            return self._csr
        csr = ops.build_csr(edge_index, num_nodes)
        if version is not None:
            self._csr_key, self._csr = (edge_index, version, num_nodes), csr
        return csr

    def clear_cache(self) -> None:
        self._csr_key = self._csr = None

    def graphed(self, max_nodes: int, max_edges: int, training: bool = False) -> "GraphedSageBlock":
        return GraphedSageBlock(self, max_nodes, max_edges, training=training)

    def forward(self, x, edge_index, batch=None):
        if len(self.convs) == 0:
            return x
        ops.check_edge_index(edge_index)
        if not isinstance(x, torch.Tensor) or x.dim() != 2:
            raise RuntimeError("SageBlock: x must be a 2-D [num_nodes, features] tensor")
        ops._require_cuda(x, "x")
        ops._require_cuda(edge_index, "edge_index")
        if edge_index.device != x.device:
            raise RuntimeError(f"SageBlock: x is on {x.device} but edge_index is on {edge_index.device}")
        if x.dtype not in (torch.float32, torch.bfloat16):
            raise RuntimeError(f"SageBlock: expected float32 (or bfloat16: bf16 feature storage) features, got {x.dtype}")
        if x.size(1) != self.convs[0].in_channels:
            raise RuntimeError(f"mat1 and mat2 shapes cannot be multiplied ({x.size(0)}x{x.size(1)} and "
                               f"{self.convs[0].in_channels}x{self.convs[0].out_channels})")
        x = x.contiguous()
        ops.index_checks.poll()
        csr = self._get_csr(edge_index, x.size(0))
        eps, slopes, drops, params = [], [], [], []
        for conv, post in zip(self.convs, self.posts):
            ln, act, drop = post[0], post[1], post[2]
            slope = float(act.negative_slope) if isinstance(act, nn.LeakyReLU) else 0.0
            for name, t in (("lin_l.weight", conv.lin_l.weight), ("lin_l.bias", conv.lin_l.bias),
                            ("lin_r.weight", conv.lin_r.weight), ("LayerNorm.weight", ln.weight), ("LayerNorm.bias", ln.bias)):
                if t.device != x.device:
                    raise RuntimeError(f"SageBlock: parameter {name} is on {t.device} but x is on {x.device}")
                if t.dtype != torch.float32:
                    raise RuntimeError(f"SageBlock: parameter {name} has dtype {t.dtype}; the kernels are float32 "
                                       "(mat1 and mat2 must have the same dtype)")
                if not t.is_contiguous():
                    raise RuntimeError(f"SageBlock: parameter {name} is not contiguous")
            p = float(drop.p) if isinstance(drop, nn.Dropout) else 0.0
            if p >= 1.0 and self.training:
                raise NotImplementedError("SageBlock: dropout p = 1 is not supported by the fused block")
            eps.append(float(ln.eps)); slopes.append(slope)
            drops.append(p if (self.training and p > 0.0) else None)
            params += [conv.lin_l.weight, conv.lin_l.bias, conv.lin_r.weight, ln.weight, ln.bias]
        return _SageBlockFn.apply(x, csr, eps, slopes, drops, *params)


class _UncachedBlock(nn.Module):

    def __init__(self, block: "SageBlock"):
        super().__init__()
        self.block = block

    def forward(self, x, edge_index):
        self.block.clear_cache()
        y = self.block(x, edge_index)
        self.block.clear_cache()
        return y


class GraphedSageBlock:

    def __init__(self, block: "SageBlock", max_nodes: int, max_edges: int, training: bool = False, device=None):
        import threading
        if len(block.convs) == 0:
            raise ValueError("GraphedSageBlock: the block has no layers")
        p0 = block.convs[0].lin_l.weight
        dev = torch.device(device) if device is not None else p0.device
        if dev.type != "cuda":
            raise RuntimeError("GraphedSageBlock: CUDA only")
        self.block, self.dev, self.training = block, dev, bool(training)
        self.max_nodes, self.max_edges = int(max_nodes), int(max_edges)
        self.fin, self.fout = block.convs[0].in_channels, block.convs[-1].out_channels
        self._lock = threading.Lock()
        with torch.cuda.device(dev):
            self._x = torch.zeros((self.max_nodes, self.fin), dtype=torch.float32, device=dev)
            self._ei = torch.full((2, self.max_edges), self.max_nodes - 1, dtype=torch.long, device=dev)
            ops.index_checks.poll(block=True)
            if self.training:
                self._x.requires_grad_(True)
                self._call = torch.cuda.make_graphed_callables(_UncachedBlock(block), (self._x, self._ei))
                return
            with torch.inference_mode():
                was_training = block.training
                block.eval()
                side = torch.cuda.Stream(device=dev)
                side.wait_stream(torch.cuda.current_stream(dev))
                with torch.cuda.stream(side):
                    for _ in range(2):
                        block.clear_cache()
                        block(self._x, self._ei)
                torch.cuda.current_stream(dev).wait_stream(side)
                torch.cuda.synchronize(dev)
                ops.index_checks.poll(block=True)
                self._graph = torch.cuda.CUDAGraph()
                block.clear_cache()
                with torch.cuda.graph(self._graph):
                    self._y = block(self._x, self._ei)
                block.clear_cache()
                block.train(was_training)

    def _fill(self, x, edge_index, N, E):
        with torch.no_grad():
            if x is not None:
                self._x[:N].copy_(x, non_blocking=True)
            self._ei[:, :E].copy_(edge_index, non_blocking=True)
            if E < self.max_edges:
                self._ei[:, E:].fill_(self.max_nodes - 1)

    def __call__(self, x: torch.Tensor, edge_index: torch.Tensor) -> torch.Tensor:
        ops.check_edge_index(edge_index)
        N, E = int(x.size(0)), int(edge_index.size(1))
        if x.dim() != 2 or x.size(1) != self.fin or x.dtype != torch.float32:
            raise RuntimeError(f"GraphedSageBlock: expected float32 x of shape [N, {self.fin}]")
        if N >= self.max_nodes or E > self.max_edges:
            raise RuntimeError(f"GraphedSageBlock: N = {N}, E = {E} exceed the bucket ({self.max_nodes - 1} nodes, "
                               f"{self.max_edges} edges)")
        with self._lock, torch.cuda.device(self.dev):
            if self.training:
                self._fill(None, edge_index, N, E)
                xs = torch.nn.functional.pad(x, (0, 0, 0, self.max_nodes - N))
                return self._call(xs, self._ei)[:N]
            with torch.inference_mode():
                self._fill(x, edge_index, N, E)
                self._graph.replay()
                return self._y[:N].clone()
```

Baseline: 2.307 billion.

## Fuse lower layer's LayerNorm/activation backward into the neighbor gather epilogue

In the multi-layer backward pass, the segment-gather that produces dx for layer l now also applies the lower layer's dropout, LeakyReLU and LayerNorm backward row-wise. It writes that layer's dz and column partials directly, so the next layer's backward consumes precomputed dz and LN partial sums instead of rereading dx. This removes a full N×F write/read round trip and a separate LN-backward pass per layer boundary. In exchange it adds new gather kernels with an LN epilogue, extra dz and partials buffers, and a path restricted to eligible shapes and the tensor-core dgrad.

```diff
diff --git a/include/sldm_sage.h b/include/sldm_sage.h
--- a/include/sldm_sage.h
+++ b/include/sldm_sage.h
@@ -101,6 +101,25 @@
                                         float* dz, float* dagg, float* dxroot,
                                         void* workspace, int64_t workspace_bytes,
                                         sldm_stream_t stream, int32_t stages);
+
+int     sldm_sage_ln_fusion_supported(int64_t N, int32_t Fin_lower, int32_t F, int32_t need_dx_lower);
+int64_t sldm_sage_ln_fusion_parts(int64_t N, int64_t E);
+int     sldm_sage_layer_backward_chain(const float* dout, const void* x, const void* agg,
+                                       const float* xhat, const float* rstd,
+                                       int64_t N, int32_t Fin, int32_t Fout,
+                                       const int32_t* csr, int64_t E,
+                                       const float* W_l, const float* W_r,
+                                       const float* ln_w, const float* ln_b, float slope,
+                                       float* dx, float* dW_l, float* db_l, float* dW_r,
+                                       float* dln_w, float* dln_b,
+                                       float* dz, float* dagg, float* dxroot,
+                                       void* workspace, int64_t workspace_bytes,
+                                       sldm_stream_t stream, int32_t stages, int32_t bf16_features,
+                                       const float* ln_parts_in,
+                                       const float* lo_xhat, const float* lo_rstd,
+                                       const float* lo_ln_w, const float* lo_ln_b, float lo_slope,
+                                       const void* lo_mask, float lo_mask_scale,
+                                       float* lo_dz, float* lo_parts);
 
 int sldm_sage_bf16_supported(int32_t Fin, int32_t Fout);
 int sldm_segment_mean_bf16(const void* src, int64_t N, int32_t F, const int32_t* csr, int64_t E, void* out,
diff --git a/sldm_gnn_b200/_lib.py b/sldm_gnn_b200/_lib.py
--- a/sldm_gnn_b200/_lib.py
+++ b/sldm_gnn_b200/_lib.py
@@ -48,6 +48,11 @@
                                            _p, _p, _p, _p, _p, _p, _p, _p, _p, _p, _i64, _p]),
     "sldm_sage_layer_backward_stages": (C.c_int, [_p, _p, _p, _p, _p, _i64, _i32, _i32, _p, _i64, _p, _p, _p, _p, _f,
                                                   _p, _p, _p, _p, _p, _p, _p, _p, _p, _p, _i64, _p, _i32]),
+    "sldm_sage_ln_fusion_supported": (C.c_int, [_i64, _i32, _i32, _i32]),
+    "sldm_sage_ln_fusion_parts": (_i64, [_i64, _i64]),
+    "sldm_sage_layer_backward_chain": (C.c_int, [_p, _p, _p, _p, _p, _i64, _i32, _i32, _p, _i64, _p, _p, _p, _p, _f,
+                                                 _p, _p, _p, _p, _p, _p, _p, _p, _p, _p, _i64, _p, _i32, _i32,
+                                                 _p, _p, _p, _p, _p, _f, _p, _f, _p, _p]),
     "sldm_sage_bf16_supported": (C.c_int, [_i32, _i32]),
     "sldm_segment_mean_bf16": (C.c_int, [_p, _i64, _i32, _p, _i64, _p, _p, _i64, _p]),
     "sldm_sage_project_forward_bf16": (C.c_int, [_p, _p, _i64, _i32, _i32, _p, _p, _p, _p, _p, _f, _f,
diff --git a/sldm_gnn_b200/csrc/capi.cu b/sldm_gnn_b200/csrc/capi.cu
--- a/sldm_gnn_b200/csrc/capi.cu
+++ b/sldm_gnn_b200/csrc/capi.cu
@@ -115,13 +115,14 @@
                                float* dln_w, float* dln_b,
                                float* dz, float* dagg, float* dxroot,
                                void* workspace, int64_t workspace_bytes,
-                               sldm_stream_t stream, int32_t stages, bool bf16_feats) {
+                               sldm_stream_t stream, int32_t stages, bool bf16_feats,
+                               const float* ln_parts_in = nullptr, const LnChain* lower = nullptr) {
   SLDM_REQUIRE(N >= 0 && E >= 0, SLDM_EINVAL, "sldm_sage_layer_backward: negative N or E");
   SLDM_REQUIRE(Fin >= 1 && Fout >= 1, SLDM_ESHAPE, "sldm_sage_layer_backward: Fin=%d Fout=%d", Fin, Fout);
   SLDM_REQUIRE(dW_l && db_l && dW_r && dln_w && dln_b, SLDM_EINVAL, "sldm_sage_layer_backward: NULL gradient output");
-  const bool need_dx = dx != nullptr;
+  const bool need_dx = dx != nullptr || lower != nullptr;
   if (N > 0) {
-    SLDM_REQUIRE(dout && x && agg && xhat && rstd && csr && W_l && W_r && ln_w && ln_b && dz, SLDM_EINVAL,
+    SLDM_REQUIRE((dout || ln_parts_in) && x && agg && xhat && rstd && csr && W_l && W_r && ln_w && ln_b && dz, SLDM_EINVAL,
                  "sldm_sage_layer_backward: NULL pointer");
     SLDM_REQUIRE(!need_dx || (dagg && dxroot), SLDM_EINVAL, "sldm_sage_layer_backward: dx needs dagg and dxroot scratch");
   }
@@ -134,8 +135,11 @@
   if (N > 0) rowptr_dst = csr + csr_layout(N, E).off[SLDM_CSR_ROWPTR_DST];
   int rc = layer_backward_launch(dout, x, agg, xhat, rstd, N, Fin, Fout, rowptr_dst, W_l, W_r, ln_w, ln_b, slope,
                                  need_dx, dW_l, db_l, dW_r, dln_w, dln_b, dz, dagg, dxroot,
-                                 static_cast<char*>(workspace) + seg_ws, workspace_bytes - seg_ws, s, stages, bf16_feats);
+                                 static_cast<char*>(workspace) + seg_ws, workspace_bytes - seg_ws, s, stages, bf16_feats,
+                                 ln_parts_in, ln_parts_in ? ln_chain_parts(N, E) : 0);
   if (rc || !need_dx || N == 0 || !(stages & SLDM_BWD_STAGE_GATHER)) return rc;
+  if (lower != nullptr)
+    return segment_gather_ln(dagg, N, Fin, csr, E, dxroot, *lower, workspace, seg_ws, s);
   return sldm_segment_reduce(dagg, N, Fin, csr, E, 1, 0, dxroot, dx,
                              workspace, seg_ws, stream);
 }
@@ -153,6 +157,49 @@
                                                sldm_stream_t stream, int32_t stages) {
   return layer_backward_impl(dout, x, agg, xhat, rstd, N, Fin, Fout, csr, E, W_l, W_r, ln_w, ln_b, slope, dx, dW_l, db_l,
                              dW_r, dln_w, dln_b, dz, dagg, dxroot, workspace, workspace_bytes, stream, stages, false);
+}
+
+static bool ln_fusion_disabled() {
+  const char* e = getenv("SLDM_DISABLE_LN_FUSION");
+  return e && e[0] == '1';
+}
+
+extern "C" int sldm_sage_ln_fusion_supported(int64_t N, int32_t Fin_lower, int32_t F, int32_t need_dx_lower) {
+  return (!ln_fusion_disabled() && N >= 1 && Fin_lower >= 1 && ln_chain_shape_ok(F) &&
+          ln_rows_path(N, Fin_lower, F, need_dx_lower != 0)) ? 1 : 0;
+}
+
+extern "C" int64_t sldm_sage_ln_fusion_parts(int64_t N, int64_t E) {
+  if (N < 0 || E < 0) return -1;
+  return N == 0 ? 0 : ln_chain_parts(N, E);
+}
+
+extern "C" int sldm_sage_layer_backward_chain(const float* dout, const void* x, const void* agg,
+                                              const float* xhat, const float* rstd,
+                                              int64_t N, int32_t Fin, int32_t Fout,
+                                              const int32_t* csr, int64_t E,
+                                              const float* W_l, const float* W_r,
+                                              const float* ln_w, const float* ln_b, float slope,
+                                              float* dx, float* dW_l, float* db_l, float* dW_r,
+                                              float* dln_w, float* dln_b,
+                                              float* dz, float* dagg, float* dxroot,
+                                              void* workspace, int64_t workspace_bytes,
+                                              sldm_stream_t stream, int32_t stages, int32_t bf16_features,
+                                              const float* ln_parts_in,
+                                              const float* lo_xhat, const float* lo_rstd,
+                                              const float* lo_ln_w, const float* lo_ln_b, float lo_slope,
+                                              const void* lo_mask, float lo_mask_scale,
+                                              float* lo_dz, float* lo_parts) {
+  SLDM_REQUIRE(!bf16_features || sldm_sage_bf16_supported(Fin, Fout), SLDM_EUNSUPPORTED,
+               "sldm_sage_layer_backward_chain: bf16 features with Fin=%d Fout=%d", Fin, Fout);
+  SLDM_REQUIRE(lo_dz == nullptr || dx == nullptr, SLDM_EINVAL,
+               "sldm_sage_layer_backward_chain: the fused gather writes the lower layer's dz instead of dx");
+  const LnChain lower{lo_xhat, lo_rstd, lo_ln_w, lo_ln_b, lo_slope, static_cast<const uint8_t*>(lo_mask), lo_mask_scale,
+                      lo_dz, lo_parts};
+  return layer_backward_impl(dout, static_cast<const float*>(x), static_cast<const float*>(agg), xhat, rstd, N, Fin,
+                             Fout, csr, E, W_l, W_r, ln_w, ln_b, slope, dx, dW_l, db_l, dW_r, dln_w, dln_b, dz, dagg,
+                             dxroot, workspace, workspace_bytes, stream, stages, bf16_features != 0, ln_parts_in,
+                             lo_dz ? &lower : nullptr);
 }
 
 extern "C" int sldm_sage_bf16_supported(int32_t Fin, int32_t Fout) {
@@ -348,33 +395,51 @@
   if (N > 0) SLDM_CUDA(cudaMemcpyAsync(out_h, act[L].p, (size_t)N * hdims[L] * 4, cudaMemcpyDeviceToHost, s));
 
   if (train) {
-    DevBuf g_cur, g_next, dz, dagg, dxroot;
+    DevBuf g_cur, g_next, dz, dz_lo, dagg, dxroot, parts, parts_lo;
     if ((rc = g_cur.alloc(N * (int64_t)Fmax * 4))) return rc;
     if ((rc = g_next.alloc(N * (int64_t)Fmax * 4))) return rc;
     if ((rc = dz.alloc(N * (int64_t)Fmax * 4))) return rc;
+    if ((rc = dz_lo.alloc(N * (int64_t)Fmax * 4))) return rc;
     if ((rc = dagg.alloc(N * (int64_t)Fmax * 4))) return rc;
     if ((rc = dxroot.alloc(N * (int64_t)Fmax * 4))) return rc;
+    const int64_t parts_bytes = sldm_sage_ln_fusion_parts(N, E) * 3 * Fmax * 4;
+    if ((rc = parts.alloc(parts_bytes))) return rc;
+    if ((rc = parts_lo.alloc(parts_bytes))) return rc;
     if (N > 0) SLDM_CUDA(cudaMemcpyAsync(g_cur.p, dout_h, (size_t)N * hdims[L] * 4, cudaMemcpyHostToDevice, s));
     std::vector<DevBuf> gpar(5 * L);
+    bool chained = false;
     for (int l = L - 1; l >= 0; --l) {
       const int Fin = hdims[l], Fout = hdims[l + 1];
       const int64_t sizes[5] = {(int64_t)Fout * Fin, Fout, (int64_t)Fout * Fin, Fout, Fout};
       for (int k = 0; k < 5; ++k) if ((rc = gpar[5 * l + k].alloc(sizes[k] * 4))) return rc;
       const bool need_dx = (l > 0) || (dx_h != nullptr);
-      rc = sldm_sage_layer_backward(g_cur.as<float>(), act[l].as<float>(), agg[l].as<float>(),
-                                    xhat[l].as<float>(), rstd[l].as<float>(), N, Fin, Fout,
-                                    d_csr.as<int32_t>(), E, par[5 * l].as<float>(), par[5 * l + 2].as<float>(),
-                                    par[5 * l + 3].as<float>(), par[5 * l + 4].as<float>(), slope,
-                                    need_dx ? g_next.as<float>() : nullptr,
-                                    gpar[5 * l].as<float>(), gpar[5 * l + 1].as<float>(), gpar[5 * l + 2].as<float>(),
-                                    gpar[5 * l + 3].as<float>(), gpar[5 * l + 4].as<float>(),
-                                    dz.as<float>(), dagg.as<float>(), dxroot.as<float>(), d_ws.p, ws_bytes, s);
+      const bool fuse = l > 0 && sldm_sage_ln_fusion_supported(N, hdims[l - 1], Fin, (l - 1 > 0) || (dx_h != nullptr));
+      const int p = 5 * (l - 1);
+      rc = sldm_sage_layer_backward_chain(chained ? nullptr : g_cur.as<float>(), act[l].p, agg[l].p,
+                                          xhat[l].as<float>(), rstd[l].as<float>(), N, Fin, Fout,
+                                          d_csr.as<int32_t>(), E, par[5 * l].as<float>(), par[5 * l + 2].as<float>(),
+                                          par[5 * l + 3].as<float>(), par[5 * l + 4].as<float>(), slope,
+                                          (need_dx && !fuse) ? g_next.as<float>() : nullptr,
+                                          gpar[5 * l].as<float>(), gpar[5 * l + 1].as<float>(), gpar[5 * l + 2].as<float>(),
+                                          gpar[5 * l + 3].as<float>(), gpar[5 * l + 4].as<float>(),
+                                          dz.as<float>(), dagg.as<float>(), dxroot.as<float>(), d_ws.p, ws_bytes, s,
+                                          SLDM_BWD_STAGE_ALL, 0, chained ? parts.as<float>() : nullptr,
+                                          fuse ? xhat[l - 1].as<float>() : nullptr, fuse ? rstd[l - 1].as<float>() : nullptr,
+                                          fuse ? par[p + 3].as<float>() : nullptr, fuse ? par[p + 4].as<float>() : nullptr,
+                                          slope, nullptr, 1.f, fuse ? dz_lo.as<float>() : nullptr,
+                                          fuse ? parts_lo.as<float>() : nullptr);
       if (rc) return rc;
       for (int k = 0; k < 5; ++k) {
         SLDM_REQUIRE(grads_h[5 * l + k] != nullptr, SLDM_EINVAL, "sage_block_host: grads[%d] is NULL", 5 * l + k);
         SLDM_CUDA(cudaMemcpyAsync(grads_h[5 * l + k], gpar[5 * l + k].p, (size_t)sizes[k] * 4, cudaMemcpyDeviceToHost, s));
       }
-      std::swap(g_cur.p, g_next.p);
+      if (fuse) {
+        std::swap(dz.p, dz_lo.p);
+        std::swap(parts.p, parts_lo.p);
+      } else {
+        std::swap(g_cur.p, g_next.p);
+      }
+      chained = fuse;
     }
     if (dx_h && N > 0) SLDM_CUDA(cudaMemcpyAsync(dx_h, g_cur.p, (size_t)N * hdims[0] * 4, cudaMemcpyDeviceToHost, s));
     SLDM_CUDA(cudaStreamSynchronize(s));
diff --git a/sldm_gnn_b200/csrc/common.cuh b/sldm_gnn_b200/csrc/common.cuh
--- a/sldm_gnn_b200/csrc/common.cuh
+++ b/sldm_gnn_b200/csrc/common.cuh
@@ -76,6 +76,16 @@
                           bool mean, const float* addend, float* out,
                           float* partials, cudaStream_t s);
 
+struct LnChain {
+  const float* xhat; const float* rstd; const float* gamma; const float* beta; float slope;
+  const uint8_t* mask; float mask_scale;
+  float* dz; float* colpart;
+};
+bool ln_chain_shape_ok(int32_t F);
+int64_t ln_chain_parts(int64_t N, int64_t E);
+int segment_gather_ln(const float* dagg, int64_t N, int32_t F, const int32_t* csr, int64_t E, const float* dxroot,
+                      const LnChain& c, void* workspace, int64_t workspace_bytes, cudaStream_t s);
+
 int project_forward_launch(const float* agg, const float* x, int64_t N, int32_t Fin, int32_t Fout,
                            const float* W_l, const float* b_l, const float* W_r,
                            const float* ln_w, const float* ln_b, float eps, float slope,
@@ -100,8 +110,10 @@
                           float* dW_l, float* db_l, float* dW_r, float* dln_w, float* dln_b,
                           float* dz, float* dagg, float* dxroot,
                           void* ws, int64_t ws_bytes, cudaStream_t s, int stages = SLDM_BWD_STAGE_ALL,
-                          bool bf16_feats = false);
+                          bool bf16_feats = false,
+                          const float* colpart_in = nullptr, int64_t ncolparts_in = 0);
 int64_t layer_backward_ws_bytes(int64_t N, int32_t Fin, int32_t Fout);
+bool ln_rows_path(int64_t N, int32_t Fin, int32_t Fout, bool need_dx);
 
 bool dgrad_tc_eligible(int64_t N, int32_t Fin, int32_t Fout, const float* dz, const float* dagg, const float* dxroot);
 int64_t dgrad_tc_ws_bytes(int32_t Fin, int32_t Fout);
diff --git a/sldm_gnn_b200/csrc/sage_bwd.cu b/sldm_gnn_b200/csrc/sage_bwd.cu
--- a/sldm_gnn_b200/csrc/sage_bwd.cu
+++ b/sldm_gnn_b200/csrc/sage_bwd.cu
@@ -491,6 +491,11 @@
 
 static bool b16(const void* p) { return (reinterpret_cast<uintptr_t>(p) & 15u) == 0; }
 
+bool ln_rows_path(int64_t N, int32_t Fin, int32_t Fout, bool need_dx) {
+  const float* a = reinterpret_cast<const float*>(256);
+  return Fout % 4 == 0 && (!need_dx || dgrad_tc_eligible(N, Fin, Fout, a, a, a));
+}
+
 template <int TX, int TN, int TM>
 static int launch_b1(int grid, size_t smem, cudaStream_t s,
                      const float* dout, const float* xhat, const float* rstd, const float* gamma,
@@ -514,7 +519,8 @@
                           bool need_dx,
                           float* dW_l, float* db_l, float* dW_r, float* dln_w, float* dln_b,
                           float* dz, float* dagg, float* dxroot,
-                          void* ws, int64_t ws_bytes, cudaStream_t s, int stages, bool bf16_feats) {
+                          void* ws, int64_t ws_bytes, cudaStream_t s, int stages, bool bf16_feats,
+                          const float* colpart_in, int64_t ncolparts_in) {
   SLDM_REQUIRE(Fin >= 1 && Fout >= 1, SLDM_ESHAPE, "backward: Fin=%d Fout=%d must be >= 1", Fin, Fout);
   SLDM_REQUIRE(!bf16_feats || N == 0 || (wgrad_bf16_eligible(N, Fin, Fout, dz, agg, x) &&
                                          (!need_dx || dgrad_tc_eligible(N, Fin, Fout, dz, dagg, dxroot))),
@@ -548,7 +554,11 @@
   int rc = SLDM_OK;
   int ncolparts = p.grid1;
   const bool ln_stream = !simt_dx && (Fout % 4 == 0) && b16(dout) && b16(xhat) && b16(dz) && b16(ln_w) && b16(ln_b);
-  if (!(stages & SLDM_BWD_STAGE_LN)) {
+  if (colpart_in != nullptr) {
+    SLDM_REQUIRE(!simt_dx, SLDM_EUNSUPPORTED, "backward: a precomputed dz needs the tensor-core data-gradient path");
+    colpart = const_cast<float*>(colpart_in);
+    ncolparts = (int)ncolparts_in;
+  } else if (!(stages & SLDM_BWD_STAGE_LN)) {
     ncolparts = ln_stream ? p.grid_ln : p.grid1;
   } else if (ln_stream) {
     ncolparts = p.grid_ln;
diff --git a/sldm_gnn_b200/csrc/segment_reduce.cu b/sldm_gnn_b200/csrc/segment_reduce.cu
--- a/sldm_gnn_b200/csrc/segment_reduce.cu
+++ b/sldm_gnn_b200/csrc/segment_reduce.cu
@@ -126,19 +126,16 @@
   for (int u = 0; u < U; ++u) { acc.x += v[u].x; acc.y += v[u].y; acc.z += v[u].z; acc.w += v[u].w; }
 }
 
-template <int LPR, int UMAX, int RW>
-__global__ void __launch_bounds__(256)
-k_segment_rows_lean(const float4* __restrict__ src, int64_t FV,
-                    const int32_t* __restrict__ rowptr, const int32_t* __restrict__ col,
-                    int64_t N, int mean, const float4* __restrict__ addend, float4* __restrict__ out) {
+template <int LPR, int UMAX, int RW, class Epi>
+__device__ __forceinline__ void lean_strip(const float4* __restrict__ src, int64_t FV,
+                                           const int32_t* __restrict__ rowptr, const int32_t* __restrict__ col,
+                                           int64_t N, int64_t strip, int* win, const Epi& epi) {
   constexpr int rw = RW;
   constexpr int RPW = 32 / LPR;
   constexpr int CH = RPW <= 4 ? 256 * RPW : 1024;
-  __shared__ int s_win[8][CH];
-  const int lane = threadIdx.x & 31, warp = threadIdx.x >> 5;
+  const int lane = threadIdx.x & 31;
   const int g = lane / LPR, lig = lane % LPR;
-  int* win = s_win[warp];
-  const int64_t wbase = ((int64_t)blockIdx.x * 8 + warp) * rw;
+  const int64_t wbase = strip * rw;
   if (wbase >= N) return;
   const int64_t wend = (wbase + rw < N) ? wbase + rw : N;
   const int64_t myrow = (wbase + lane < wend) ? wbase + lane : wend;
@@ -170,6 +167,7 @@
     const int64_t row = wbase + rfirst + g;
     const int deg = end - beg;
     if (row >= wend || deg > SLDM_HUB_DEGREE) continue;
+    const auto pre = epi.preload(row, cvalid);
     float4 acc = make_float4(0.f, 0.f, 0.f, 0.f);
     if (beg >= ws && end <= ws + CH) {
       const int* w = win + (beg - ws);
@@ -189,6 +187,15 @@
         acc.x += v.x; acc.y += v.y; acc.z += v.z; acc.w += v.w;
       }
     }
+    epi(row, deg, cvalid, acc, pre);
+  }
+}
+
+struct LeanStore {
+  int64_t FV; int lig; int mean; const float4* __restrict__ addend; float4* __restrict__ out;
+  struct Nothing {};
+  __device__ __forceinline__ Nothing preload(int64_t, bool) const { return {}; }
+  __device__ __forceinline__ void operator()(int64_t row, int deg, bool cvalid, float4 acc, Nothing) const {
     if (cvalid) {
       if (mean && deg > 1) {
         if ((deg & (deg - 1)) == 0) {
@@ -202,6 +209,139 @@
       out[row * FV + lig] = acc;
     }
   }
+};
+
+template <int LPR, int UMAX, int RW>
+__global__ void __launch_bounds__(256)
+k_segment_rows_lean(const float4* __restrict__ src, int64_t FV,
+                    const int32_t* __restrict__ rowptr, const int32_t* __restrict__ col,
+                    int64_t N, int mean, const float4* __restrict__ addend, float4* __restrict__ out) {
+  constexpr int RPW = 32 / LPR;
+  constexpr int CH = RPW <= 4 ? 256 * RPW : 1024;
+  __shared__ int s_win[8][CH];
+  const int warp = threadIdx.x >> 5;
+  const LeanStore epi{FV, (int)(threadIdx.x & 31) % LPR, mean, addend, out};
+  lean_strip<LPR, UMAX, RW>(src, FV, rowptr, col, N, (int64_t)blockIdx.x * 8 + warp, s_win[warp], epi);
+}
+
+struct LnBwdArgs {
+  const float4* __restrict__ addend;
+  const float4* __restrict__ xhat;
+  const float* __restrict__ rstd;
+  const float4* __restrict__ gamma;
+  const float4* __restrict__ beta;
+  float slope;
+  const uchar4* __restrict__ mask;
+  float mask_scale;
+  float fF;
+  float4* __restrict__ dz;
+};
+
+__device__ __forceinline__ void ln_bwd_add_pg_pb(float4* pg, float4* pb, const float* dy, const float* hh) {
+  float4 v = *pg, w = *pb;
+  v.x = fmaf(dy[0], hh[0], v.x); v.y = fmaf(dy[1], hh[1], v.y); v.z = fmaf(dy[2], hh[2], v.z); v.w = fmaf(dy[3], hh[3], v.w);
+  w.x += dy[0]; w.y += dy[1]; w.z += dy[2]; w.w += dy[3];
+  *pg = v; *pb = w;
+}
+
+struct LnRowIn { float4 dxroot, xhat; float rstd; uchar4 mask; };
+
+__device__ __forceinline__ LnRowIn ln_bwd_row_load(const LnBwdArgs& a, int64_t FV, int lig, int64_t row, bool cvalid) {
+  LnRowIn in;
+  in.dxroot = in.xhat = f4zero();
+  in.mask = make_uchar4(0, 0, 0, 0);
+  if (cvalid) {
+    in.dxroot = ldg_stream_f4(a.addend + row * FV + lig);
+    in.xhat = ldg_stream_f4(a.xhat + row * FV + lig);
+    if (a.mask != nullptr) in.mask = a.mask[row * FV + lig];
+  }
+  in.rstd = __ldg(a.rstd + row);
+  return in;
+}
+
+__device__ __forceinline__ void ln_bwd_row(const LnBwdArgs& a, int64_t FV, int lig, int64_t row, bool cvalid,
+                                           float4 acc, const LnRowIn& in, float4* pg, float4* pb, float4* pdb) {
+  float4 d = in.dxroot, g = f4zero(), be = f4zero();
+  const float4 h = in.xhat;
+  if (cvalid) {
+    Vec<float4>::add(d, acc);
+    if (a.mask != nullptr) {
+      const uchar4 m = in.mask;
+      d.x = (float)m.x * d.x * a.mask_scale; d.y = (float)m.y * d.y * a.mask_scale;
+      d.z = (float)m.z * d.z * a.mask_scale; d.w = (float)m.w * d.w * a.mask_scale;
+    }
+    g = __ldg(a.gamma + lig);
+    be = __ldg(a.beta + lig);
+  }
+  const float rs = in.rstd;
+  const float* dd = reinterpret_cast<const float*>(&d);
+  const float* hh = reinterpret_cast<const float*>(&h);
+  const float* gg = reinterpret_cast<const float*>(&g);
+  const float* bb = reinterpret_cast<const float*>(&be);
+  float dy[4], tt[4];
+  float s1 = 0.f, s2 = 0.f;
+#pragma unroll
+  for (int e = 0; e < 4; ++e) {
+    const float y = fmaf(hh[e], gg[e], bb[e]);
+    dy[e] = y > 0.f ? dd[e] : dd[e] * a.slope;
+    tt[e] = dy[e] * gg[e];
+    s1 += tt[e];
+    s2 = fmaf(tt[e], hh[e], s2);
+  }
+  if (cvalid) ln_bwd_add_pg_pb(pg, pb, dy, hh);
+#pragma unroll
+  for (int o = 16; o > 0; o >>= 1) {
+    s1 += __shfl_xor_sync(0xffffffffu, s1, o);
+    s2 += __shfl_xor_sync(0xffffffffu, s2, o);
+  }
+  const float c1 = __fdiv_rn(s1, a.fF), c2 = __fdiv_rn(s2, a.fF);
+  if (cvalid) {
+    float4 o4;
+    float* oo = reinterpret_cast<float*>(&o4);
+#pragma unroll
+    for (int e = 0; e < 4; ++e) oo[e] = rs * (tt[e] - c1 - hh[e] * c2);
+    a.dz[row * FV + lig] = o4;
+    float4 v = *pdb;
+    v.x += o4.x; v.y += o4.y; v.z += o4.z; v.w += o4.w;
+    *pdb = v;
+  }
+}
+
+__device__ __forceinline__ void ln_bwd_store_parts(const float* cp, int F, float* __restrict__ colpart) {
+  __syncthreads();
+  for (int idx = threadIdx.x; idx < 3 * F; idx += 256) {
+    const int which = idx / F, c = idx % F;
+    float s = 0.f;
+#pragma unroll
+    for (int w = 0; w < 8; ++w) s += cp[(w * 3 + which) * 128 + c];
+    colpart[(int64_t)blockIdx.x * 3 * F + idx] = s;
+  }
+}
+
+struct LeanLnEpi {
+  LnBwdArgs a; int64_t FV; int lig; float4* part;
+  __device__ __forceinline__ LnRowIn preload(int64_t row, bool cvalid) const {
+    return ln_bwd_row_load(a, FV, lig, row, cvalid);
+  }
+  __device__ __forceinline__ void operator()(int64_t row, int, bool cvalid, float4 acc, const LnRowIn& in) const {
+    ln_bwd_row(a, FV, lig, row, cvalid, acc, in, part, part + 32, part + 64);
+  }
+};
+
+template <int UMAX, int RW>
+__global__ void __launch_bounds__(256, 5)
+k_segment_rows_lean_ln(const float4* __restrict__ src, int64_t FV,
+                       const int32_t* __restrict__ rowptr, const int32_t* __restrict__ col,
+                       int64_t N, LnBwdArgs a, float* __restrict__ colpart) {
+  __shared__ int s_win[8][256];
+  __shared__ float4 s_part[8][3][32];
+  const int lane = threadIdx.x & 31, warp = threadIdx.x >> 5;
+  float4* part = &s_part[warp][0][lane];
+  part[0] = part[32] = part[64] = f4zero();
+  const LeanLnEpi epi{a, FV, lane, part};
+  for (int64_t b = blockIdx.x; b * 8 * RW < N; b += gridDim.x)
+    lean_strip<32, UMAX, RW>(src, FV, rowptr, col, N, b * 8 + warp, s_win[warp], epi);
+  ln_bwd_store_parts(reinterpret_cast<const float*>(s_part), (int)FV * 4, colpart);
 }
 
 template <typename VT, int LPR, int VPL, int UNR>
@@ -269,6 +409,35 @@
   }
 }
 
+__global__ void __launch_bounds__(256)
+k_segment_hub_finalize_ln(const float4* __restrict__ partials, int64_t FV,
+                          const int4* __restrict__ hub_list, const int32_t* __restrict__ hub_count,
+                          int cap, LnBwdArgs a, float* __restrict__ colpart) {
+  __shared__ float4 s_part[8][3][32];
+  const int n = min(*hub_count, cap);
+  const int lane = threadIdx.x & 31, warp = threadIdx.x >> 5;
+  const bool cvalid = lane < FV;
+  float4 pg = f4zero(), pb = f4zero(), pdb = f4zero();
+  for (int64_t c = (int64_t)blockIdx.x * 8 + warp; c < n; c += (int64_t)gridDim.x * 8) {
+    const int4 ent = hub_list[c];
+    if (ent.y != 0) continue;
+    const LnRowIn in = ln_bwd_row_load(a, FV, lane, ent.x, cvalid);
+    float4 s = f4zero();
+    if (cvalid) {
+      s = partials[c * FV + lane];
+      for (int j = 1; j < ent.z; ++j) Vec<float4>::add(s, partials[(c + j) * FV + lane]);
+    }
+    ln_bwd_row(a, FV, lane, ent.x, cvalid, s, in, &pg, &pb, &pdb);
+  }
+  s_part[warp][0][lane] = pg; s_part[warp][1][lane] = pb; s_part[warp][2][lane] = pdb;
+  ln_bwd_store_parts(reinterpret_cast<const float*>(s_part), (int)FV * 4, colpart);
+}
+
+static int seg_lean_mode() {
+  static const int lean = [] { const char* e = getenv("SLDM_SEG_LEAN"); return e ? atoi(e) : 4; }();
+  return lean;
+}
+
 template <typename VT, int LPR, int VPL, int UNR>
 static int launch_all(const float* src, int64_t N, int64_t FV,
                       const int32_t* rowptr, const int32_t* col,
@@ -280,7 +449,7 @@
   VT* vpart = reinterpret_cast<VT*>(partials);
   const int64_t grid = ceil_div<int64_t>(N, kRowsPerCta);
   if constexpr (std::is_same<VT, float4>::value && VPL == 1) {
-    static const int lean = [] { const char* e = getenv("SLDM_SEG_LEAN"); return e ? atoi(e) : 4; }();
+    const int lean = seg_lean_mode();
     constexpr int RW = (LPR == 32) ? 8 : 32;
     const int64_t lgrid = ceil_div<int64_t>(N, 8 * RW);
     if (lean == 4 || lean == 1)
@@ -326,6 +495,59 @@
   }
   if (F <= 32) return launch_all<float, 32, 1, 8>(src, N, F, rowptr, col, hub_list, hub_count, hub_cap, mean, addend, out, partials, s);
   return launch_all<float, 32, 4, 4>(src, N, F, rowptr, col, hub_list, hub_count, hub_cap, mean, addend, out, partials, s);
+}
+
+constexpr int kLnRW = 8;
+
+static int64_t ln_lean_grid(int64_t N) {
+  return std::max<int64_t>(1, std::min<int64_t>(ceil_div<int64_t>(N, 8 * kLnRW), (int64_t)num_sms() * 8));
+}
+static int64_t ln_hub_grid(int64_t E) {
+  return E > SLDM_HUB_DEGREE ? std::min<int64_t>(ceil_div<int64_t>(hub_capacity(E), 8), 64) : 0;
+}
+
+bool ln_chain_shape_ok(int32_t F) { return F % 4 == 0 && F > 64 && F <= 128 && seg_lean_mode() != 0; }
+
+int64_t ln_chain_parts(int64_t N, int64_t E) { return ln_lean_grid(N) + ln_hub_grid(E); }
+
+int segment_gather_ln(const float* dagg, int64_t N, int32_t F, const int32_t* csr, int64_t E, const float* dxroot,
+                      const LnChain& c, void* workspace, int64_t workspace_bytes, cudaStream_t s) {
+  SLDM_REQUIRE(ln_chain_shape_ok(F), SLDM_EUNSUPPORTED, "fused LayerNorm gather: F=%d not in (64, 128] or F %% 4 != 0", F);
+  SLDM_REQUIRE(aligned16(dagg) && aligned16(dxroot) && aligned16(c.xhat) && aligned16(c.gamma) && aligned16(c.beta) &&
+               aligned16(c.dz) && aligned16(workspace) && (reinterpret_cast<uintptr_t>(c.mask) & 3u) == 0,
+               SLDM_EUNSUPPORTED, "fused LayerNorm gather: buffers must be 16-byte aligned (the mask 4-byte aligned)");
+  SLDM_REQUIRE(c.xhat && c.rstd && c.gamma && c.beta && c.dz && c.colpart, SLDM_EINVAL, "fused LayerNorm gather: NULL pointer");
+  const int64_t need = sldm_segment_workspace_bytes(N, E, F);
+  SLDM_REQUIRE(workspace_bytes >= need && (workspace != nullptr || need == 0), SLDM_EWORKSPACE,
+               "fused LayerNorm gather: workspace %lld < %lld bytes", (long long)workspace_bytes, (long long)need);
+  if (N == 0) return SLDM_OK;
+  const int64_t FV = F / 4;
+  const LnBwdArgs a{reinterpret_cast<const float4*>(dxroot), reinterpret_cast<const float4*>(c.xhat), c.rstd,
+                    reinterpret_cast<const float4*>(c.gamma), reinterpret_cast<const float4*>(c.beta), c.slope,
+                    reinterpret_cast<const uchar4*>(c.mask), c.mask_scale, (float)F, reinterpret_cast<float4*>(c.dz)};
+  CsrLayout L = csr_layout(N, E);
+  const int32_t* meta = csr + L.off[SLDM_CSR_META];
+  const int32_t* rowptr = csr + L.off[SLDM_CSR_ROWPTR_SRC];
+  const int32_t* col = csr + L.off[SLDM_CSR_COL_DST];
+  const int4* hub = reinterpret_cast<const int4*>(csr + L.off[SLDM_CSR_HUB_SRC]);
+  const float4* src = reinterpret_cast<const float4*>(dagg);
+  const unsigned g1 = (unsigned)ln_lean_grid(N);
+  if (seg_lean_mode() == 8)
+    k_segment_rows_lean_ln<8, kLnRW><<<g1, 256, 0, s>>>(src, FV, rowptr, col, N, a, c.colpart);
+  else
+    k_segment_rows_lean_ln<4, kLnRW><<<g1, 256, 0, s>>>(src, FV, rowptr, col, N, a, c.colpart);
+  SLDM_LAUNCH_CHECK("k_segment_rows_lean_ln");
+  if (E > SLDM_HUB_DEGREE) {
+    const int cap = (int)hub_capacity(E);
+    float4* part = static_cast<float4*>(workspace);
+    const int gc = (int)std::min<int64_t>(cap, (int64_t)num_sms() * 8);
+    k_segment_hub_chunks<float4, 32, 1, 8><<<gc, 256, 0, s>>>(src, FV, rowptr, col, hub, meta + 1, cap, part);
+    SLDM_LAUNCH_CHECK("k_segment_hub_chunks");
+    k_segment_hub_finalize_ln<<<(unsigned)ln_hub_grid(E), 256, 0, s>>>(part, FV, hub, meta + 1, cap, a,
+                                                                        c.colpart + (int64_t)g1 * 3 * F);
+    SLDM_LAUNCH_CHECK("k_segment_hub_finalize_ln");
+  }
+  return SLDM_OK;
 }
 
 }
diff --git a/sldm_gnn_b200/ops.py b/sldm_gnn_b200/ops.py
--- a/sldm_gnn_b200/ops.py
+++ b/sldm_gnn_b200/ops.py
@@ -248,7 +248,8 @@
     return x, out, agg, xhat, rstd
 
 
-def backward_buffers(N: int, Fin: int, Fout: int, E: int, dev, need_dx: bool, grad_out=None) -> dict:
+def backward_buffers(N: int, Fin: int, Fout: int, E: int, dev, need_dx: bool, grad_out=None, dz=None,
+                     dx: bool = True) -> dict:
     with torch.cuda.device(dev):
         f32 = dict(dtype=torch.float32, device=dev)
         if grad_out is not None:
@@ -256,9 +257,9 @@
         else:
             b = dict(dW_l=torch.empty((Fout, Fin), **f32), dW_r=torch.empty((Fout, Fin), **f32),
                      db_l=torch.empty((Fout,), **f32), dln_w=torch.empty((Fout,), **f32), dln_b=torch.empty((Fout,), **f32))
-        b.update(dz=torch.empty((N, Fout), **f32), dx=None, dagg=None, dxroot=None)
+        b.update(dz=dz if dz is not None else torch.empty((N, Fout), **f32), dx=None, dagg=None, dxroot=None)
         if need_dx:
-            b.update(dx=torch.empty((N, Fin), **f32), dagg=torch.empty((N, Fin), **f32),
+            b.update(dx=torch.empty((N, Fin), **f32) if dx else None, dagg=torch.empty((N, Fin), **f32),
                      dxroot=torch.empty((N, Fin), **f32))
         wsb = int(lib.sldm_sage_layer_bwd_workspace_bytes(N, E, Fin, Fout))
         b["wsb"] = wsb
@@ -297,3 +298,55 @@
         else:
             launch(stages)
     return b["dx"], b["dW_l"], b["db_l"], b["dW_r"], b["dln_w"], b["dln_b"]
+
+
+def ln_fusion_supported(N: int, Fin_lower: int, F: int, need_dx_lower: bool) -> bool:
+    return bool(lib.sldm_sage_ln_fusion_supported(int(N), int(Fin_lower), int(F), int(bool(need_dx_lower))))
+
+
+def layer_backward_chained(dout, x, agg, xhat, rstd, csr: Csr, W_l, W_r, ln_w, ln_b, slope: float, need_dx: bool,
+                           ln_in: dict | None = None, lower: dict | None = None, on_param_grads=None, grad_out=None):
+    N, Fin = x.shape
+    Fout = W_l.shape[0]
+    dev = x.device
+    if ln_in is None and dout.dtype != torch.float32:
+        raise RuntimeError(f"layer_backward_chained: dout is {dout.dtype}")
+    if x.dtype != agg.dtype:
+        raise RuntimeError(f"layer_backward_chained: x is {x.dtype}, agg is {agg.dtype}")
+    dout = None if ln_in is not None else dout.contiguous()
+    need_dx = need_dx or lower is not None
+    b = backward_buffers(N, Fin, Fout, csr.E, dev, need_dx, grad_out, dz=None if ln_in is None else ln_in["dz"],
+                         dx=lower is None)
+    out = None
+    lo = (None,) * 5 + (0.0, None, 1.0, None, None)
+    with torch.cuda.device(dev):
+        if lower is not None:
+            parts = int(lib.sldm_sage_ln_fusion_parts(N, csr.E))
+            out = dict(dz=torch.empty((N, Fin), dtype=torch.float32, device=dev),
+                       parts=torch.empty((max(parts, 1), 3 * Fin), dtype=torch.float32, device=dev))
+            mask = lower.get("mask")
+            if mask is not None and (mask.dtype != torch.bool or not mask.is_contiguous()):
+                raise RuntimeError("layer_backward_chained: the lower layer's dropout mask must be a contiguous bool tensor")
+            lo = (None, lower["xhat"].data_ptr(), lower["rstd"].data_ptr(), lower["ln_w"].data_ptr(),
+                  lower["ln_b"].data_ptr(), float(lower["slope"]), _ptr(mask), float(lower.get("mask_scale", 1.0)),
+                  out["dz"].data_ptr(), out["parts"].data_ptr())
+
+        def launch(mask):
+            check(lib.sldm_sage_layer_backward_chain(
+                _ptr(dout), x.data_ptr(), agg.data_ptr(), xhat.data_ptr(), rstd.data_ptr(), N, Fin, Fout,
+                csr.buf.data_ptr(), csr.E, W_l.data_ptr(), W_r.data_ptr(), ln_w.data_ptr(), ln_b.data_ptr(), float(slope),
+                _ptr(b["dx"]), b["dW_l"].data_ptr(), b["db_l"].data_ptr(), b["dW_r"].data_ptr(), b["dln_w"].data_ptr(),
+                b["dln_b"].data_ptr(), b["dz"].data_ptr(), _ptr(b["dagg"]), _ptr(b["dxroot"]), b["ws"].data_ptr(),
+                b["wsb"], _stream(dev), int(mask), int(x.dtype == torch.bfloat16),
+                None if ln_in is None else ln_in["parts"].data_ptr(), *lo[1:]))
+
+        if on_param_grads is not None:
+            launch(_lib.BWD_STAGE_ALL & ~_lib.BWD_STAGE_GATHER)
+            ev = torch.cuda.Event()
+            ev.record(torch.cuda.current_stream(dev))
+            on_param_grads(ev)
+            if need_dx and N > 0:
+                launch(_lib.BWD_STAGE_GATHER)
+        else:
+            launch(_lib.BWD_STAGE_ALL)
+    return b["dx"], b["dW_l"], b["db_l"], b["dW_r"], b["dln_w"], b["dln_b"], out
diff --git a/sldm_gnn_b200/sageblock.py b/sldm_gnn_b200/sageblock.py
--- a/sldm_gnn_b200/sageblock.py
+++ b/sldm_gnn_b200/sageblock.py
@@ -85,23 +85,33 @@
             sink = active_wrapper()
         grads = [None] * (5 * L)
         g = dout if dout.dtype == torch.float32 else dout.float()
+        ln_in = None
         for l in range(L - 1, -1, -1):
             h, agg, xhat, rstd, mask = keep[5 * l:5 * l + 5]
             W_l, _, W_r, ln_w, ln_b = params[5 * l:5 * l + 5]
-            if mask is not None:
-                g = torch.ops.aten.native_dropout_backward(g, mask, 1.0 / (1.0 - ctx.drops[l]))
-            g = g.contiguous()
+            if ln_in is None:
+                if mask is not None:
+                    g = torch.ops.aten.native_dropout_backward(g, mask, 1.0 / (1.0 - ctx.drops[l]))
+                g = g.contiguous()
             need_dx = l > 0 or ctx.needs_input_grad[0]
+            lower = None
+            if l > 0:
+                h_lo, _, xhat_lo, rstd_lo, mask_lo = keep[5 * (l - 1):5 * l]
+                if ops.ln_fusion_supported(h.size(0), h_lo.size(1), h.size(1), l - 1 > 0 or ctx.needs_input_grad[0]):
+                    lower = dict(xhat=xhat_lo, rstd=rstd_lo, ln_w=params[5 * (l - 1) + 3], ln_b=params[5 * (l - 1) + 4],
+                                 slope=ctx.slopes[l - 1], mask=mask_lo,
+                                 mask_scale=1.0 / (1.0 - ctx.drops[l - 1]) if mask_lo is not None else 1.0)
             claim = sink.claim(params[5 * l:5 * l + 5]) if sink is not None else None
             if claim is not None:
                 bi, views = claim
-                dx = ops.layer_backward(g, h, agg, xhat, rstd, ctx.csr, W_l, W_r, ln_w, ln_b, ctx.slopes[l], need_dx,
-                                        grad_out=views, on_param_grads=lambda ev, bi=bi: sink.bucket_ready(bi, ev))[0]
+                res = ops.layer_backward_chained(g, h, agg, xhat, rstd, ctx.csr, W_l, W_r, ln_w, ln_b, ctx.slopes[l],
+                                                 need_dx, ln_in=ln_in, lower=lower, grad_out=views,
+                                                 on_param_grads=lambda ev, bi=bi: sink.bucket_ready(bi, ev))
             else:
-                dx, dW_l, db_l, dW_r, dln_w, dln_b = ops.layer_backward(
-                    g, h, agg, xhat, rstd, ctx.csr, W_l, W_r, ln_w, ln_b, ctx.slopes[l], need_dx)
-                grads[5 * l:5 * l + 5] = [dW_l, db_l, dW_r, dln_w, dln_b]
-            g = dx
+                res = ops.layer_backward_chained(g, h, agg, xhat, rstd, ctx.csr, W_l, W_r, ln_w, ln_b, ctx.slopes[l],
+                                                 need_dx, ln_in=ln_in, lower=lower)
+                grads[5 * l:5 * l + 5] = res[1:6]
+            g, ln_in = res[0], res[6]
         return (g, None, None, None, None, *grads)
 
 
```

Result: no change. 2.324 billion (median of 6 runs) (+0.8%).
